# Zoz4/Pooraytracer

Hardware: AMD Instinct MI355X
Metric: Mrays/s (primary+secondary) at fixed spp; s/frame in ms_per_step (higher is better)
Workload: dtype f64; 1 GPU; cornell-box (synthetic stand-in, 20492 tris, 4-wide BVH 6148 nodes) 1024x1024 spp=500 depth=20 rr=0.8 bSampleLights seed=1; parallelism=32x32 tiles dealt diagonally over 1 GPU(s), rays_per_frame=2362685805

## Files before the change

pooraytracer_amd/csrc/prt_api.cpp:

```cpp
#include <hip/hip_runtime.h>
#include <rccl/rccl.h>

#include <algorithm>
#include <atomic>
#include <cmath>
#include <cstddef>
#include <cstdio>
#include <cstdlib>
#include <chrono>
#include <cstring>
#include <limits>
#include <map>
#include <memory>
#include <mutex>
#include <new>
#include <string>
#include <type_traits>
#include <vector>

#include "mesh_topology.h"
#include "prt_host.h"
#include "prt_launch.h"

namespace {
// ... 55 lines not shown
        if (e != hipSuccess || cap >= bytes) return e;
        if (done && (e = hipEventSynchronize(done.get())) != hipSuccess) return e;
        p.reset();
        cap = 0;
        if ((e = dev_alloc(p, bytes)) == hipSuccess) cap = bytes;
        return e;
    }
    hipError_t used(hipStream_t st) {
        const hipError_t e = done ? hipSuccess : make_event(done, hipEventDisableTiming);
        return e == hipSuccess ? hipEventRecord(done.get(), st) : e;
    }
    template <typename T>
    T* get() const { return static_cast<T*>(p.get()); }
};

struct Staging {
    std::vector<DevBuf<>> bufs;
    hipError_t e = hipSuccess;
    void* out(size_t bytes) {
        DevBuf<> b;
        if (e == hipSuccess) e = dev_alloc(b, std::max<size_t>(bytes, 16));
        bufs.push_back(std::move(b));
        return bufs.back().get();
    }
    void* in(const void* src, size_t bytes) {
        if (!src) return nullptr;
        void* d = out(bytes);
        if (e == hipSuccess) e = hipMemcpy(d, src, bytes, hipMemcpyHostToDevice);
        return d;
    }
    void sync(hipEvent_t ev = nullptr) {
        if (e == hipSuccess) e = ev ? hipEventSynchronize(ev) : hipDeviceSynchronize();
    }
    void down(void* dst, const void* src, size_t bytes) {
        if (e == hipSuccess) e = hipMemcpy(dst, src, bytes, hipMemcpyDeviceToHost);
    }
    int status(const std::string& who) const { return e == hipSuccess ? PRT_OK : hip_fail(who, e); }
};

template <typename R>
struct KernelConfig {
    DSceneT<R> d{};
    int blocks_per_cu[3] = {0, 0, 0};
    int blocks_per_cu_rays = 0;
    int light_lds = 0, ltri_lds = 0, mat_lds = 0;
    int stack_depth = PRT_STACK_DEPTH;
};
}

extern "C" int prt_dev_hooks(void) { return PRT_DEV_HOOKS; }

#if PRT_DEV_HOOKS
static std::atomic<int> g_render_form{PRT_RENDER_FORM_UNKNOWN};
static void note_render_form(bool plain) { g_render_form = plain ? PRT_RENDER_FORM_PLAIN : PRT_RENDER_FORM_GENERIC; }
extern "C" int prt_last_render_form(void) { return g_render_form; }
#else
static void note_render_form(bool) {}
extern "C" int prt_last_render_form(void) { return PRT_RENDER_FORM_UNKNOWN; }
#endif

#define PRT_HIP_AS(who, call)                                                                           \
    do {                                                                                                \
        const hipError_t e_ = (call);                                                                   \
        if (e_ != hipSuccess) return hip_fail(who, e_);                                                 \
    } while (0)
#define PRT_HIP(call) PRT_HIP_AS(#call, call)

struct PrtScene {
    std::vector<prt::HostTri> tris;
    std::vector<DMaterial> mats;
    std::vector<DTexture> texs;
    std::vector<double> texels_lin;
    size_t n_texel_reals = 0;
    size_t tex_footprint_bytes = 0;
    uint32_t tex_layouts = 0;
    prt::LightTree lights;
    prt::BuiltBVH bvh;
    std::vector<uint64_t> mesh_first;
    std::vector<int32_t> mesh_mat;
    std::vector<int32_t> light_meshes;
    bool explicit_lights = false;
    bool device_bvh = false;
    uint64_t generation = 0;
    PrtBvhInfo bvh_info{};
    int device = -1;
    int n_cu = 0;
    int blocks_wanted = 0;
    int feat = 0;
    KernelConfig<double> k64;
    KernelConfig<float> k32;
    bool f32_ready = false;
    int stack_need = PRT_STACK_DEPTH;
    const DNode* d_nodes_shallow = nullptr;
    uint32_t n_nodes_shallow = 0;
    std::vector<DevBuf<>> allocs;
    const uint32_t* d_order = nullptr;
    struct Refit {
        float* d_tbox = nullptr;
        uint32_t *d_parent = nullptr, *d_cnt = nullptr;
        uint32_t *d_parent_sh = nullptr, *d_cnt_sh = nullptr;
        void* d_scratch = nullptr;
        prt::RefitCheck* d_check = nullptr;
        double* d_sah = nullptr;
        Event ev0, ev1, ev2;
        Event done;
        bool pending = false;
        uint64_t count = 0;
    } refit;
    Scratch refit_in;
    bool host_stale = false;
    Event feat_done;
    bool feat_pending = false;
    bool dynamic_lights = false;
    struct LightArrays {
        void *nodes = nullptr, *tris = nullptr, *tab = nullptr, *nodes32 = nullptr, *tris32 = nullptr;
        size_t cap_nodes = 0, cap_tris = 0, cap_tab = 0, cap_nodes32 = 0, cap_tris32 = 0;
    };
    LightArrays light_res, light_spare;
    bool distance_queries = false;
    DTriCorners* d_corners = nullptr;
    bool signed_queries = false;
    prt::DSignedTables sq;
    size_t signed_bytes = 0;
    bool winding_queries = false;
    prt::DWindingMoment* d_moments = nullptr;
    struct LightUpdate {
        double* d_gather = nullptr;
        std::vector<double> h_gather;
        Scratch tmp;
        prt::LightTree next;
        prt::LightTablePlan plan;
        std::vector<uint32_t> words;
        uint32_t flag = 0;
        std::vector<DLightNodeT<float>> ln32;
        std::vector<DLightTriT<float>> lt32;
        std::vector<int32_t> prims;
        std::vector<prt::HostTri> saved;
        bool staged = false;
        bool staged_relaid = false, staged_dropped = false, staged_tables = false;
        Event g0, g1, t0, t1;
        bool tables_timed = false;
        uint64_t count = 0;
        double host_tree_ms = 0.0, gather_ms = 0.0;
        double staged_host_tree_ms = 0.0, staged_gather_ms = 0.0;
        int fail_alloc_at = -1, n_allocs = 0;
        uint32_t tables_dropped = 0, relaid = 0;
    } lu;
    hipError_t after_refit(hipStream_t st) const {
        return refit.pending ? hipStreamWaitEvent(st, refit.done.get(), 0) : hipSuccess;
    }
    struct CallSlot {
        DevBuf<DCounters> d_ctr;
        Scratch partial;
        Event ev0, ev1;
        Event done;
        bool timed = false;
        bool counted = false;
        uint64_t samples = 0;
        hipError_t start(hipStream_t st) {
            const hipError_t e = hipMemsetAsync(d_ctr.get(), 0, sizeof(DCounters), st);
            return e == hipSuccess ? hipEventRecord(ev0.get(), st) : e;
        }
        hipError_t stop(hipStream_t st) { return hipEventRecord(ev1.get(), st); }
        hipError_t finish(hipStream_t st, bool count, uint64_t n) {
            const hipError_t e = hipEventRecord(done.get(), st);
            if (e == hipSuccess) {
// ... 119 lines not shown
        sq = prt::DSignedTables();
        signed_bytes = 0;
        d_moments = nullptr;
        refit = Refit();
        light_res = light_spare = LightArrays();
        lu = LightUpdate();
        refit_in = Scratch();
        multi_fb = Scratch();
        sort = Scratch();
        dn = Scratch();
        for (CallSlot& q : slots) q = CallSlot();
        k64 = KernelConfig<double>();
        k32 = KernelConfig<float>();
        device = -1;
        f32_ready = false;
    }
};

static int check_node_count(const std::string& who, size_t n_nodes) {
    if (const char* e = dev_env("PRT_TEST_CLAIM_NODES")) n_nodes = (size_t)std::strtoull(e, nullptr, 10);
    std::string err;
    if (!prt::node_count_ok(n_nodes, &err)) return fail(PRT_E_LIMIT, who + ": " + err);
    return PRT_OK;
}

struct BvhDumpHeader {
    uint32_t magic, version;
    uint64_t n_tris, n_nodes;
    uint32_t built_on_device, depth;
    int32_t stack_need;
    uint32_t node_bytes;
    float grid_origin[3], grid_step[3], coord_scale;
    uint32_t zero;
};
static_assert(sizeof(BvhDumpHeader) == 72, "dump header layout");

static int dump_bvh(const char* path, const PrtScene* s, const DNode* nodes, size_t n_nodes, const uint32_t* order,
                    int stack_need) {
    BvhDumpHeader h;
    std::memset(&h, 0, sizeof(h));
    h.magic = 0x48564250u;
    h.version = 1;
    h.n_tris = s->tris.size();
    h.n_nodes = n_nodes;
    h.built_on_device = s->bvh_info.built_on_device;
    h.depth = s->bvh_info.depth;
    h.stack_need = stack_need;
    h.node_bytes = sizeof(DNode);
    for (int a = 0; a < 3; ++a) {
        h.grid_origin[a] = s->bvh.grid_origin[a];
        h.grid_step[a] = s->bvh.grid_step[a];
    }
    h.coord_scale = s->bvh.coord_scale;
    FILE* f = std::fopen(path, "wb");
    if (!f) return fail(PRT_E_INVALID, std::string("PRT_TEST_DUMP_BVH: cannot open ") + path);
    bool ok = std::fwrite(&h, sizeof(h), 1, f) == 1;
    ok = ok && std::fwrite(nodes, sizeof(DNode), n_nodes, f) == n_nodes;
    ok = ok && std::fwrite(order, sizeof(uint32_t), s->tris.size(), f) == s->tris.size();
    ok = (std::fclose(f) == 0) && ok;
    return ok ? PRT_OK : fail(PRT_E_INVALID, std::string("PRT_TEST_DUMP_BVH: cannot write ") + path);
}

template <typename T, typename U>
static void conv_arr(T* o, const U* a, int n) {
    for (int i = 0; i < n; ++i) o[i] = (T)a[i];
}

static void size_tables(const PrtScene* s, int budget, size_t mat_bytes, size_t ltri_bytes, size_t lnode_bytes, int* mat, int* ltri, int* light) {
    *mat = *ltri = *light = 0;
    const bool off = dev_env("PRT_TUNE_NO_LDS") && std::atoi(dev_env("PRT_TUNE_NO_LDS"));
    if (off || s->mats.empty() || s->mats.size() * mat_bytes > 8192 || (int)(s->mats.size() * mat_bytes) > budget) return;
    *mat = (int)s->mats.size();
    budget -= *mat * (int)mat_bytes;
    if (!s->lights.tris.empty() && s->lights.tris.size() <= 32 && (int)(s->lights.tris.size() * ltri_bytes) <= budget) {
        *ltri = (int)s->lights.tris.size();
        budget -= *ltri * (int)ltri_bytes;
    }
    *light = (int)std::min<size_t>(s->lights.nodes.size(), (size_t)(std::max(budget, 0) / (int)lnode_bytes));
    if (const char* e = dev_env("PRT_TUNE_LIGHT_LDS")) *light = std::min(*light, std::max(0, std::atoi(e)));
    if (const char* e = dev_env("PRT_TUNE_LTRI_LDS")) if (!std::atoi(e)) *ltri = 0;
}

template <typename R>
static bool frame_plain(const PrtScene* s, const KernelConfig<R>& k, bool count, bool rays, int jitter, int scramble, int sample_lights) {
    const auto plain = std::is_same<R, double>::value ? prt::render_plain : prt32::render_plain;
    return plain(s->feat, count, rays, k.d.n_lights, k.ltri_lds, jitter, scramble, sample_lights);
}
static bool generic_forced() {
    const char* e = dev_env("PRT_TUNE_GENERIC");
    return e && std::atoi(e);
}

template <typename R>
static int size_kernels(const PrtScene* s, KernelConfig<R>& k, bool drop_tables) {
    constexpr bool f64 = std::is_same<R, double>::value;
    const auto lds_budget = f64 ? prt::render_lds_budget : prt32::render_lds_budget;
    const auto table_bytes = f64 ? prt::render_table_bytes : prt32::render_table_bytes;
    const auto blocks_per_cu = f64 ? prt::render_blocks_per_cu : prt32::render_blocks_per_cu;
    size_tables(s, lds_budget(s->feat, k.stack_depth), sizeof(DMaterialT<R>), sizeof(DLightTriT<R>), sizeof(DLightNodeT<R>),
                &k.mat_lds, &k.ltri_lds, &k.light_lds);
    const bool pad = k.d.tri_stride == PRT_TRI_PAD_STRIDE(R) && sizeof(DTriT<R>) != PRT_TRI_PAD_STRIDE(R);
    const bool extra = !s->lights.tab.empty() || k.d.tex_compact != 0;
    auto blocks = [&](bool count, size_t tables, bool plain = false) { return blocks_per_cu(count, s->feat, tables, k.stack_depth, pad, extra, false, plain); };
    const size_t tables = table_bytes(k.light_lds, k.mat_lds, k.ltri_lds);
    k.blocks_per_cu[0] = blocks(false, tables);
    k.blocks_per_cu[2] = frame_plain(s, k, false, false, 0, 0, 1) ? blocks(false, tables, true) : 0;
    const int wanted = drop_tables && tables != 0 ? blocks(false, 0) : k.blocks_per_cu[0];
    if (k.blocks_per_cu[0] < wanted || (k.blocks_per_cu[2] && k.blocks_per_cu[2] < wanted)) {
        k.mat_lds = k.ltri_lds = k.light_lds = 0;
        k.blocks_per_cu[0] = wanted;
        k.blocks_per_cu[2] = 0;
    }
    k.blocks_per_cu[1] = blocks(true, table_bytes(k.light_lds, k.mat_lds, k.ltri_lds));
    if (dev_env("PRT_TUNE_VERBOSE")) {
        if (f64)
            std::fprintf(stderr, "[prt] fp64 render kernels: %d blocks per CU, LDS tables: %d materials, %d light triangles, %d light nodes\n",
                         k.blocks_per_cu[0], k.mat_lds, k.ltri_lds, k.light_lds);
        else
            std::fprintf(stderr, "[prt] fp32 render kernels: %d blocks per CU, stacks %d, LDS tables: %d materials, %d light triangles, %d light nodes\n",
                         k.blocks_per_cu[0], k.stack_depth, k.mat_lds, k.ltri_lds, k.light_lds);
    }
    return wanted;
}

static void size_kernels_again(PrtScene* s) {
    s->k64.blocks_per_cu_rays = 0;
    s->blocks_wanted = size_kernels(s, s->k64, true);
    if (s->f32_ready) {
        s->k32.blocks_per_cu_rays = 0;
        size_kernels(s, s->k32, false);
    }
}

template <typename R>
static int rays_blocks_per_cu(const PrtScene* s, KernelConfig<R>& k) {
    if (!k.blocks_per_cu_rays) {
        constexpr bool f64 = std::is_same<R, double>::value;
        const size_t tables = (f64 ? prt::render_table_bytes : prt32::render_table_bytes)(k.light_lds, k.mat_lds, k.ltri_lds);
        const bool pad = k.d.tri_stride == PRT_TRI_PAD_STRIDE(R) && sizeof(DTriT<R>) != PRT_TRI_PAD_STRIDE(R);
        k.blocks_per_cu_rays = (f64 ? prt::render_blocks_per_cu : prt32::render_blocks_per_cu)(false, s->feat, tables, k.stack_depth, pad, true, true, false);
    }
    return k.blocks_per_cu_rays;
}

template <typename R>
static uint32_t render_variant(const PrtScene* s, const KernelConfig<R>& k) {
    const bool llds = k.mat_lds != 0 || k.ltri_lds != 0 || k.light_lds != 0;
    const bool pad = k.d.tri_stride == PRT_TRI_PAD_STRIDE(R) && sizeof(DTriT<R>) != PRT_TRI_PAD_STRIDE(R);
    const bool extra = k.d.light_tab != nullptr || k.d.tex_compact != 0;
    return PRT_VARIANT_VALID | ((uint32_t)s->feat & PRT_VARIANT_PERM_MASK) | (llds ? PRT_VARIANT_LLDS : 0u) |
           (pad ? PRT_VARIANT_PAD : 0u) | (extra ? PRT_VARIANT_EXTRA : 0u);
}

struct TileLayout {
    int width, height, tile, tiles_x, tiles_y, n_tiles, rank, nranks, owned_tiles;
    uint64_t items_per_chunk;
    TileLayout(const PrtCamera& c, const PrtRenderParams& p) : width(c.width), height(c.height), rank(p.rank), nranks(p.nranks) {
        tile = p.tile_size > 0 ? p.tile_size : 32;
        tile = std::max(8, (tile + 7) / 8 * 8);
        tiles_x = (width + tile - 1) / tile;
        tiles_y = (height + tile - 1) / tile;
        n_tiles = tiles_x * tiles_y;
        owned_tiles = n_tiles > rank ? (n_tiles - rank + nranks - 1) / nranks : 0;
        items_per_chunk = (uint64_t)owned_tiles * tile * tile;
    }
    bool owns(int x, int y) const {
        const int tx = x / tile, ty = y / tile;
        const int kx = ((tx - 3 * ty) % tiles_x + tiles_x) % tiles_x;
        return (ty * tiles_x + kx) % nranks == rank;
    }
    uint64_t owned_pixels() const {
        uint64_t px = 0;
        for (int k = rank; k < n_tiles; k += nranks) {
            const int ty = k / tiles_x, tx = (k - ty * tiles_x + 3 * ty) % tiles_x;
            px += (uint64_t)std::max(0, std::min(tile, width - tx * tile)) * (uint64_t)std::max(0, std::min(tile, height - ty * tile));
        }
        return px;
    }
    void set(DRenderParams& P) const {
        P.tile = tile; P.tiles_x = tiles_x; P.tiles_y = tiles_y; P.n_tiles = n_tiles;
        P.rank = rank; P.nranks = nranks; P.owned_tiles = owned_tiles; P.items_per_chunk = items_per_chunk;
    }
};

#ifndef PRT_CHAIN_MIN_DEFAULT
#define PRT_CHAIN_MIN_DEFAULT 8
#endif
static DRenderParams base_params(const PrtScene* s, const PrtRenderParams* p) {
    DRenderParams P;
// ... 15 lines not shown
    P.stack_depth = PRT_STACK_DEPTH;
    return P;
}

static DRenderParamsT<float> to_f32(const DRenderParams& P, const KernelConfig<float>& k) {
    static_assert(sizeof(DRenderParamsT<float>) == 400, "DRenderParamsT changed: convert its new fields here");
    DRenderParamsT<float> o;
    std::memset(&o, 0, sizeof(o));
    o.spp = P.spp; o.max_depth = P.max_depth; o.sample_lights = P.sample_lights; o.chunks = P.chunks;
    o.rr = (float)P.rr; o.inv_rr = (float)P.inv_rr;
    conv_arr(o.background, P.background, 3);
    o.seed_key = P.seed_key;
    o.tile = P.tile; o.tiles_x = P.tiles_x; o.tiles_y = P.tiles_y; o.n_tiles = P.n_tiles;
    o.rank = P.rank; o.nranks = P.nranks; o.owned_tiles = P.owned_tiles; o.jitter = P.jitter;
    o.keep = P.keep; o.leaf_batch = P.leaf_batch; o.inner_min = P.inner_min; o.scramble = P.scramble; o.cached_min = P.cached_min; o.chain_min = P.chain_min;
    o.light_lds = k.light_lds; o.mat_lds = k.mat_lds; o.ltri_lds = k.ltri_lds;
    o.stack_depth = k.stack_depth;
    o.items_per_chunk = P.items_per_chunk; o.n_items = P.n_items;
    std::memcpy(o.chunk_begin, P.chunk_begin, sizeof(P.chunk_begin));
    return o;
}
static DCameraT<float> to_f32(const DCamera& C) {
    DCameraT<float> o;
    conv_arr(o.center, C.center, 3); conv_arr(o.pixel00, C.pixel00, 3);
    conv_arr(o.du, C.du, 3); conv_arr(o.dv, C.dv, 3);
    o.width = C.width; o.height = C.height;
    return o;
}

extern "C" {

int prt_abi_version(void) { return PRT_ABI_VERSION; }
const char* prt_last_error(void) { return g_err.c_str(); }

int prt_device_count(int* n) {
    if (!n) return fail(PRT_E_INVALID, "prt_device_count: null argument");
    int c = 0;
    hipError_t e = hipGetDeviceCount(&c);
    if (e != hipSuccess) {
        *n = 0;
        return fail(PRT_E_NO_DEVICE, std::string("hipGetDeviceCount: ") + hipGetErrorString(e));
    }
    *n = c;
    return PRT_OK;
}

int prt_scene_create(const PrtSceneDesc* desc, PrtScene** out) {
    if (!desc || !out) return fail(PRT_E_INVALID, "prt_scene_create: null argument");
    *out = nullptr;
    if (desc->n_tris && !desc->vertices) return fail(PRT_E_INVALID, "prt_scene_create: vertices is null");
    if (desc->n_meshes && (!desc->mesh_first_tri || !desc->mesh_material))
        return fail(PRT_E_INVALID, "prt_scene_create: mesh arrays are null");
    if (desc->n_materials && !desc->materials) return fail(PRT_E_INVALID, "prt_scene_create: materials is null");
    if (desc->n_textures && !desc->textures) return fail(PRT_E_INVALID, "prt_scene_create: textures is null");
    if (desc->n_meshes) {
        if (desc->mesh_first_tri[0] != 0 || desc->mesh_first_tri[desc->n_meshes] != desc->n_tris)
            return fail(PRT_E_INVALID, "prt_scene_create: mesh_first_tri must start at 0 and end at n_tris");
        for (uint32_t m = 0; m < desc->n_meshes; ++m) {
            if (desc->mesh_first_tri[m] > desc->mesh_first_tri[m + 1])
                return fail(PRT_E_INVALID, "prt_scene_create: mesh_first_tri must be ascending");
            if (desc->mesh_material[m] < 0 || (uint32_t)desc->mesh_material[m] >= desc->n_materials)
                return fail(PRT_E_INVALID, "prt_scene_create: mesh_material out of range");
        }
    } else if (desc->n_tris) {
        return fail(PRT_E_INVALID, "prt_scene_create: triangles without meshes");
    }
    if (desc->n_light_meshes && !desc->light_meshes) return fail(PRT_E_INVALID, "prt_scene_create: light_meshes is null");
    for (uint32_t i = 0; i < (desc->light_meshes ? desc->n_light_meshes : 0u); ++i)
        if (desc->light_meshes[i] < 0 || (uint32_t)desc->light_meshes[i] >= desc->n_meshes)
            return fail(PRT_E_INVALID, "prt_scene_create: light_meshes entry out of range");
    for (uint32_t i = 0; i < desc->n_materials; ++i) {
        const PrtMaterial& m = desc->materials[i];
        if (m.type < PRT_MAT_LAMBERTIAN || m.type > PRT_MAT_EMPTY)
            return fail(PRT_E_INVALID, "prt_scene_create: unknown material type");
        if (m.texture >= (int32_t)desc->n_textures) return fail(PRT_E_INVALID, "prt_scene_create: texture index out of range");
    }
    for (uint64_t i = 0; i < desc->n_tris * 9; ++i)
        if (!(std::fabs(desc->vertices[i]) <= 1e18))
            return fail(PRT_E_INVALID, "prt_scene_create: vertex coordinate is not finite (or beyond 1e18)");
    PrtScene* s = new (std::nothrow) PrtScene();
    if (!s) return fail(PRT_E_OOM, "prt_scene_create: out of host memory");
    try {
        prt::setup_triangles(*desc, s->tris);
        s->mesh_first.assign(desc->mesh_first_tri, desc->mesh_first_tri + (desc->n_meshes ? desc->n_meshes + 1 : 0));
        s->mesh_mat.assign(desc->mesh_material, desc->mesh_material + desc->n_meshes);
        s->explicit_lights = desc->light_meshes != nullptr;
        if (s->explicit_lights) s->light_meshes.assign(desc->light_meshes, desc->light_meshes + desc->n_light_meshes);
        prt::setup_materials(*desc, s->mats);
        s->texs.resize(desc->n_textures);
        for (uint32_t i = 0; i < desc->n_textures; ++i) {
            const PrtTexture& t = desc->textures[i];
            DTexture& o = s->texs[i];
            o.width = t.width;
            o.height = t.height;
            o.channels = t.channels;
            o.has_data = (t.data && t.width > 0 && t.height > 0 && t.channels > 0) ? 1 : 0;
            o.offset = s->texels_lin.size();
            if (o.has_data) {
                double lut[256];
                for (int b = 0; b < 256; ++b) {
                    const double c = (1.0 / 255.0) * b;
                    lut[b] = (c <= 0.04045) ? c * (1. / 12.92) : std::pow((c + 0.055) * (1. / 1.055), 2.4);
                }
                const size_t npx = (size_t)t.width * t.height;
                s->texels_lin.reserve(s->texels_lin.size() + npx * 3);
                for (size_t i = 0; i < npx; ++i) {
                    const uint8_t* px = t.data + i * t.channels;
                    if (t.channels >= 3) {
                        s->texels_lin.push_back(lut[px[0]]);
                        s->texels_lin.push_back(lut[px[1]]);
                        s->texels_lin.push_back(lut[px[2]]);
                    } else {
                        const double g = (1.0 / 255.0) * px[0];
                        s->texels_lin.insert(s->texels_lin.end(), {g, g, g});
                    }
                }
            }
        }
        prt::build_light_tree(*desc, s->tris, s->mats, s->lights);
        s->device_bvh = (desc->flags & PRT_SCENE_DEVICE_BVH) && s->tris.size() >= 2;
        if (!s->device_bvh) {
            std::string err;
            const auto t0 = std::chrono::steady_clock::now();
            if (!prt::build_bvh(s->tris, s->bvh, &err)) {
                delete s;
                return fail(PRT_E_LIMIT, "prt_scene_create: " + err);
            }
            if (const int rc = check_node_count("prt_scene_create", s->bvh.nodes.size())) {
                delete s;
                return rc;
            }
            s->bvh_info.build_ms = std::chrono::duration<double, std::milli>(std::chrono::steady_clock::now() - t0).count();
        }
    } catch (const std::bad_alloc&) {
        delete s;
        return fail(PRT_E_OOM, "prt_scene_create: out of host memory");
    } catch (const std::exception& e) {
        delete s;
        return fail(PRT_E_INVALID, std::string("prt_scene_create: ") + e.what());
    }
    s->last.bvh_nodes = s->bvh.nodes.size();
    s->last.bvh_depth = s->bvh.depth;
    s->bvh_info.n_nodes = s->bvh.nodes.size();
    s->bvh_info.depth = s->bvh.depth;
    if (const char* p = dev_env("PRT_TEST_DUMP_BVH"))
        if (!s->device_bvh) {
            const int rc = dump_bvh(p, s, s->bvh.nodes.data(), s->bvh.nodes.size(), s->bvh.order.data(), s->bvh.stack_need);
            if (rc != PRT_OK) {
                delete s;
                return rc;
            }
        }
    *out = s;
    return PRT_OK;
}

void prt_scene_destroy(PrtScene* s) {
    if (!s) return;
    s->release();
    delete s;
}

int prt_scene_bvh_info(const PrtScene* s, PrtBvhInfo* out) {
    if (!s || !out) return fail(PRT_E_INVALID, "prt_scene_bvh_info: null argument");
    *out = s->bvh_info;
    out->node_bytes = (uint32_t)sizeof(DNode);
// ... 300 lines not shown
            for (int y0 = 0; y0 < t.height; ++y0)
                for (int x0 = 0; x0 < t.width; ++x0) {
                    const int x1 = std::min(x0 + 1, t.width - 1), y1 = std::min(y0 + 1, t.height - 1);
                    double* o = quads.data() + at;
                    const int tap[4][2] = {{x0, y0}, {x1, y0}, {x0, y1}, {x1, y1}};
                    for (int k = 0; k < 4; ++k) std::memcpy(o + 3 * k, px + ((size_t)tap[k][1] * t.width + tap[k][0]) * 3, 24);
                    at += 16;
                }
        }
        d.tex_compact = compact ? 1u : 0u;
        s->tex_footprint_bytes = compact ? 0 : cells_all * 16 * sizeof(double);
        s->tex_layouts = cells_all == 0 ? 0u : (compact ? 2u : 1u);
        s->n_texel_reals = quads.size();
        if ((rc = s->up(qt, &d.textures))) return rc;
        if ((rc = s->up(quads, &d.texels_lin))) return rc;
    }
    if ((rc = s->up(s->lights.nodes, &d.light_nodes))) return rc;
    d.light_tab = nullptr;
    if (!s->lights.tab.empty() && (rc = s->up(s->lights.tab, &d.light_tab))) return rc;
    if ((rc = s->up(s->lights.tris, &d.light_tris))) return rc;
    s->light_res.nodes = const_cast<DLightNode*>(d.light_nodes);
    s->light_res.tris = const_cast<DLightTri*>(d.light_tris);
    s->light_res.tab = const_cast<uint32_t*>(d.light_tab);
    s->light_res.cap_nodes = s->lights.nodes.size();
    s->light_res.cap_tris = s->lights.tris.size();
    s->light_res.cap_tab = s->lights.tab.size();
    d.light_root = s->lights.root;
    d.n_lights = (int32_t)s->lights.tris.size();
    d.light_area = s->lights.area;
    d.n_tris = (uint32_t)n;
    for (PrtScene::CallSlot& q : s->slots) {
        PRT_HIP_AS("hipMalloc", dev_alloc(q.d_ctr, sizeof(DCounters)));
        PRT_HIP(hipMemset(q.d_ctr.get(), 0, sizeof(DCounters)));
        PRT_HIP(make_event(q.ev0, hipEventDefault));
        PRT_HIP(make_event(q.ev1, hipEventDefault));
        PRT_HIP(make_event(q.done, hipEventDisableTiming));
    }
    s->feat = 0;
    for (const DMaterial& m : s->mats) {
        if (m.texture >= 0) s->feat |= 1;
        if (m.type == PRT_MAT_PHONG) s->feat |= 2;
        if (m.type == PRT_MAT_COOKTORRANCE) s->feat |= 4;
    }
    if (const char* e = dev_env("PRT_TUNE_FEAT")) s->feat |= std::atoi(e);
    s->feat = prt::render_permutation(s->feat);
    {
        int need = s->bvh.stack_need;
        if (s->bvh_info.built_on_device)
            PRT_HIP_AS("hipMemcpy(hn.data(), d.nodes, (size_t)d.n_nodes * sizeof(DNode), hipMemcpyDeviceToHost)",
                       device_tree_stack_need(d.nodes, d.n_nodes, &need));
        if (dump_path && (rc = dump_bvh(dump_path, s, dump_nodes.data(), dump_nodes.size(), dump_order.data(), need))) return rc;
        s->set_stack_need(need);
        s->d_nodes_shallow = nullptr;
        s->n_nodes_shallow = 0;
        if (dev_env("PRT_TUNE_VERBOSE")) std::fprintf(stderr, "[prt] tree needs %d stack entries\n", s->stack_need);
    }
    static_assert(sizeof(DLightNode) == 16 && sizeof(DLightTri) % 16 == 0, "LDS staging copies 16-byte pieces");
    s->blocks_wanted = size_kernels(s, s->k64, true);
    if (s->distance_queries && (rc = corners_from_host(s, "prt_scene_upload"))) return rc;
    if (s->signed_queries && (rc = signed_from_host(s, "prt_scene_upload"))) return rc;
    if (s->winding_queries && (rc = winding_from_resident(s, "prt_scene_upload"))) return rc;
    return PRT_OK;
}

static void light_desc(const PrtScene* s, PrtSceneDesc& d) {
    std::memset(&d, 0, sizeof(d));
    d.n_tris = s->tris.size();
    d.n_meshes = (uint32_t)s->mesh_mat.size();
    d.mesh_first_tri = s->mesh_first.data();
    d.mesh_material = s->mesh_mat.data();
    static const int32_t none = 0;
    d.light_meshes = s->explicit_lights ? (s->light_meshes.empty() ? &none : s->light_meshes.data()) : nullptr;
    d.n_light_meshes = (uint32_t)s->light_meshes.size();
}

int prt_scene_update_vertices(PrtScene* s, const double* vertices, const double* normals) {
    if (!s || (!vertices && !s->tris.empty())) return fail(PRT_E_INVALID, "prt_scene_update_vertices: null argument");
    for (size_t i = 0; i < s->tris.size() * 9; ++i)
        if (!(std::fabs(vertices[i]) <= 1e18)) return fail(PRT_E_INVALID, "prt_scene_update_vertices: vertex coordinate is not finite (or beyond 1e18)");
    ++s->generation;
    try {
        prt::update_triangles(vertices, normals, s->tris);
        s->host_stale = false;
        PrtSceneDesc d;
        light_desc(s, d);
        s->lights = prt::LightTree();
        prt::build_light_tree(d, s->tris, s->mats, s->lights);
        if (s->device >= 0 && s->tris.size() >= 2) {
            s->device_bvh = true;
        } else if (!s->device_bvh) {
            std::string err;
            const auto t0 = std::chrono::steady_clock::now();
            if (!prt::build_bvh(s->tris, s->bvh, &err)) return fail(PRT_E_LIMIT, "prt_scene_update_vertices: " + err);
            s->bvh_info.build_ms = std::chrono::duration<double, std::milli>(std::chrono::steady_clock::now() - t0).count();
            s->last.bvh_nodes = s->bvh_info.n_nodes = s->bvh.nodes.size();
            s->last.bvh_depth = s->bvh_info.depth = s->bvh.depth;
            if (const char* p = dev_env("PRT_TEST_DUMP_BVH")) {
                const int rc = dump_bvh(p, s, s->bvh.nodes.data(), s->bvh.nodes.size(), s->bvh.order.data(), s->bvh.stack_need);
                if (rc != PRT_OK) return rc;
            }
        }
    } catch (const std::bad_alloc&) {
        return fail(PRT_E_OOM, "prt_scene_update_vertices: out of host memory");
    }
    if (s->device >= 0) return prt_scene_upload(s, s->device);
    return PRT_OK;
}

static int ensure_f32_impl(PrtScene* s);
static int f32_stack_depth(int need) {
    int depth = need <= PRT_STACK_SHALLOW ? PRT_STACK_SHALLOW : PRT_STACK_DEPTH;
    if (const char* e = dev_env("PRT_TUNE_STACK32")) depth = std::max(need, std::min(PRT_STACK_DEPTH, std::atoi(e)));
    return depth;
}
static void light_tables_f32(const prt::LightTree& lights, std::vector<DLightNodeT<float>>& ln, std::vector<DLightTriT<float>>& lt) {
    ln.resize(lights.nodes.size());
    for (size_t i = 0; i < ln.size(); ++i) {
        std::memset(&ln[i], 0, sizeof(ln[i]));
        ln[i].left_area = (float)lights.nodes[i].left_area;
        ln[i].left = lights.nodes[i].left;
        ln[i].right = lights.nodes[i].right;
    }
    lt.resize(lights.tris.size());
    for (size_t i = 0; i < lt.size(); ++i) {
        const DLightTri& a = lights.tris[i];
        DLightTriT<float>& o = lt[i];
        std::memset(&o, 0, sizeof(o));
        conv_arr(o.v0, a.v0, 3); conv_arr(o.v1, a.v1, 3); conv_arr(o.v2, a.v2, 3); conv_arr(o.n, a.n, 3);
        o.area = (float)a.area; o.material = a.material; o.prim = a.prim; o.pdf = (float)a.pdf;
    }
}
static int ensure_f32(PrtScene* s) {
    if (s->f32_ready) return PRT_OK;
    const size_t mark = s->allocs.size();
    const int rc = ensure_f32_impl(s);
    if (rc != PRT_OK) {
        KeepError keep;
        s->allocs.resize(mark);
        s->k32 = KernelConfig<float>();
        s->light_res.nodes32 = s->light_res.tris32 = nullptr;
        s->light_res.cap_nodes32 = s->light_res.cap_tris32 = 0;
    }
    return rc;
}
static int ensure_f32_impl(PrtScene* s) {
    const DScene& d = s->k64.d;
    KernelConfig<float>& k = s->k32;
    DSceneT<float>& f = k.d;
    const size_t n = d.n_tris;
    const uint32_t stride = d.tri_stride == sizeof(DTriT<double>) ? (uint32_t)sizeof(DTriT<float>) : PRT_TRI_PAD_STRIDE(float);
    void *t = nullptr, *sh = nullptr, *tx = nullptr;
    int rc;
    if ((rc = s->alloc(n * (size_t)stride, &t)) || (rc = s->alloc(n * sizeof(DTriShadeT<float>), &sh)) ||
        (rc = s->alloc(s->n_texel_reals * sizeof(float), &tx)))
        return rc;
    PRT_HIP(s->after_refit(nullptr));
    prt32::launch_convert_tris(d.tris, d.tri_stride, (uint32_t)n, t, stride, nullptr);
    prt32::launch_convert_shade(d.shade, (uint32_t)n, static_cast<DTriShadeT<float>*>(sh), nullptr);
    prt32::launch_convert_reals(d.texels_lin, s->n_texel_reals, static_cast<float*>(tx), nullptr);
    PRT_HIP(hipGetLastError());
    std::vector<DMaterialT<float>> mats(s->mats.size());
    for (size_t i = 0; i < mats.size(); ++i) {
        const DMaterial& a = s->mats[i];
        DMaterialT<float>& o = mats[i];
        std::memset(&o, 0, sizeof(o));
        o.type = a.type; o.texture = a.texture;
// ... 21 lines not shown
    {
        int need = s->stack_need;
        if ((rc = s->shallow_resident())) return rc;
        if (s->d_nodes_shallow) need = std::min(need, PRT_STACK_SHALLOW);
        s->share_with_f32();
        k.stack_depth = f32_stack_depth(need);
        if (dev_env("PRT_TUNE_VERBOSE")) std::fprintf(stderr, "[prt] fp32 tables: tree needs %d stack entries, using %d\n", need, k.stack_depth);
    }
    size_kernels(s, k, false);
    s->f32_ready = true;
    return PRT_OK;
}

static int require_uploaded(PrtScene* s, const char* who) {
    if (!s) return fail(PRT_E_INVALID, std::string(who) + ": null scene");
    if (s->device < 0) return fail(PRT_E_NO_DEVICE, std::string(who) + ": scene is not uploaded to a HIP device (no CPU path exists)");
    PRT_HIP(hipSetDevice(s->device));
    return PRT_OK;
}

namespace {
float f32_round_down(double v) {
    float f = (float)v;
    if ((double)f > v) f = std::nextafter(f, -std::numeric_limits<float>::infinity());
    return f;
}
float f32_round_up(double v) {
    float f = (float)v;
    if ((double)f < v) f = std::nextafter(f, std::numeric_limits<float>::infinity());
    return f;
}
size_t round16(size_t b) { return (b + 15) & ~(size_t)15; }
}

static hipError_t refit_baseline(PrtScene* s, hipStream_t st) {
    const PrtScene::Refit& R = s->refit;
    const DScene& d = s->k64.d;
    prt::launch_refit_parents(d.nodes, d.n_nodes, R.d_parent, st);
    prt::launch_refit_sah(d.nodes, d.n_nodes, d.grid_origin, d.grid_step, R.d_scratch, R.d_sah, st);
    return hipMemcpyAsync(R.d_sah + 1, R.d_sah, sizeof(double), hipMemcpyDeviceToDevice, st);
}

static int refit_prepare(PrtScene* s, hipStream_t st) {
    PrtScene::Refit& R = s->refit;
    const DScene& d = s->k64.d;
    int rc;
    if (!R.d_check) {
        void *tbox, *parent, *cnt, *scratch, *check, *sah;
        if ((rc = s->alloc((size_t)d.n_tris * 6 * sizeof(float), &tbox)) || (rc = s->alloc((size_t)d.n_nodes * sizeof(uint32_t), &parent)) ||
            (rc = s->alloc(round16((size_t)d.n_nodes * sizeof(uint32_t)), &cnt)) || (rc = s->alloc(prt::refit_scratch_bytes(), &scratch)) ||
            (rc = s->alloc(2 * sizeof(double), &sah)) || (rc = s->alloc(sizeof(prt::RefitCheck), &check)))
            return rc;
        PRT_HIP(make_event(R.ev0, hipEventDefault));
        PRT_HIP(make_event(R.ev1, hipEventDefault));
        PRT_HIP(make_event(R.ev2, hipEventDefault));
        PRT_HIP(make_event(R.done, hipEventDisableTiming));
        if ((rc = s->shallow_resident())) return rc;
        R.d_tbox = static_cast<float*>(tbox);
        R.d_parent = static_cast<uint32_t*>(parent);
        R.d_cnt = static_cast<uint32_t*>(cnt);
        R.d_scratch = scratch;
        R.d_sah = static_cast<double*>(sah);
        PRT_HIP_AS("hipMemcpyAsync(R.d_sah + 1, R.d_sah, sizeof(double), hipMemcpyDeviceToDevice, st)", refit_baseline(s, st));
        PRT_HIP(hipGetLastError());
        R.d_check = static_cast<prt::RefitCheck*>(check);
    }
    if (s->d_nodes_shallow && !R.d_parent_sh) {
        void *parent, *cnt;
        if ((rc = s->alloc((size_t)s->n_nodes_shallow * sizeof(uint32_t), &parent)) ||
            (rc = s->alloc(round16((size_t)s->n_nodes_shallow * sizeof(uint32_t)), &cnt)))
            return rc;
        prt::launch_refit_parents(s->d_nodes_shallow, s->n_nodes_shallow, static_cast<uint32_t*>(parent), st);
        PRT_HIP(hipGetLastError());
        R.d_cnt_sh = static_cast<uint32_t*>(cnt);
        R.d_parent_sh = static_cast<uint32_t*>(parent);
    }
    return PRT_OK;
}

struct RefitGridHost {
    float origin[3], step[3], root_hi[3];
    double origin_d[3], delta;
    bool lights_moved = false;
};

static int refit_begin(PrtScene* s, const std::string& who, const double* d_verts, const double* d_normals, hipStream_t st,
                       RefitGridHost& g) {
    DScene& d = s->k64.d;
    const uint32_t n = d.n_tris;
    PrtScene::Refit& R = s->refit;
    if (!d_verts) return fail(PRT_E_INVALID, who + ": null vertices");
    PRT_HIP_AS(who, s->after_refit(st));
    {
        const size_t mark = s->allocs.size();
        const bool fresh = !R.d_check;
        const DNode* const shallow_before = s->d_nodes_shallow;
        const uint32_t n_shallow_before = s->n_nodes_shallow;
        const int rc = refit_prepare(s, st);
        if (rc != PRT_OK) {
            KeepError keep;
            if (fresh) {
                (void)hipDeviceSynchronize();
                s->allocs.resize(mark);
                R = PrtScene::Refit();
                s->d_nodes_shallow = shallow_before;
                s->n_nodes_shallow = n_shallow_before;
            }
            return rc;
        }
    }
    PrtScene::LightUpdate& U = s->lu;
    const size_t nl = (size_t)d.n_lights;
    const bool gather = s->dynamic_lights && nl > 0;
    if (gather && !U.d_gather) {
        PRT_HIP_AS(who, make_event(U.g0, hipEventDefault));
        PRT_HIP_AS(who, make_event(U.g1, hipEventDefault));
        PRT_HIP_AS(who, make_event(U.t0, hipEventDefault));
        PRT_HIP_AS(who, make_event(U.t1, hipEventDefault));
        void* p = nullptr;
        if (const int rc = s->alloc(nl * 18 * sizeof(double), &p)) return rc;
        U.d_gather = static_cast<double*>(p);
    }
    if (gather) {
        try {
            U.h_gather.resize(nl * 18);
        } catch (const std::bad_alloc&) {
            return fail(PRT_E_OOM, who + ": out of host memory");
        }
        PRT_HIP_AS(who, hipEventRecord(U.g0.get(), st));
    }
    prt::launch_refit_check(d_verts, n, d.light_tris, (uint32_t)d.n_lights, R.d_scratch, R.d_check, st, d_normals,
                            gather ? U.d_gather : nullptr, gather ? U.d_gather + nl * 9 : nullptr);
    PRT_HIP_AS(who, hipGetLastError());
    prt::RefitCheck c;
    PRT_HIP_AS(who, hipMemcpyAsync(&c, R.d_check, sizeof(c), hipMemcpyDeviceToHost, st));
    if (gather) {
        PRT_HIP_AS(who, hipMemcpyAsync(U.h_gather.data(), U.d_gather, nl * (d_normals ? 18 : 9) * sizeof(double), hipMemcpyDeviceToHost, st));
        PRT_HIP_AS(who, hipEventRecord(U.g1.get(), st));
    }
    PRT_HIP_AS(who, hipEventRecord(R.done.get(), st));
    R.pending = true;
    PRT_HIP_AS(who, hipStreamSynchronize(st));
    if (c.flags & 1u) return fail(PRT_E_INVALID, who + ": vertex coordinate is not finite (or beyond 1e18)");
    if ((c.flags & 2u) && !s->dynamic_lights)
        return fail(PRT_E_INVALID, who + ": a vertex of a light mesh moved; emitters stay in place under a refit (the light tree is not "
                                         "rebuilt) - use prt_scene_update_vertices");
    g.lights_moved = (c.flags & 2u) != 0;
    const double extent = std::max(1.0, std::max(c.hi[0] - c.lo[0], std::max(c.hi[1] - c.lo[1], c.hi[2] - c.lo[2])));
    g.delta = 1e-9 * extent + 256.0 * std::numeric_limits<double>::epsilon() * c.scale;
    for (int a = 0; a < 3; ++a) {
        g.origin[a] = f32_round_down(c.lo[a] - 2.0 * g.delta);
        g.origin_d[a] = (double)g.origin[a];
        g.root_hi[a] = f32_round_up((c.hi[a] + g.delta) - g.origin_d[a]);
    }
    const float zero[3] = {0.f, 0.f, 0.f};
    float rel0[3];
    prt::quant_grid(zero, g.root_hi, false, rel0, g.step);
    return PRT_OK;
}

static int light_grow(PrtScene* s, void*& p, size_t& cap, size_t need, size_t elem) {
    if (p && cap >= need) return PRT_OK;
    if (s->lu.n_allocs++ == s->lu.fail_alloc_at) return fail(PRT_E_OOM, "light update: injected allocation failure (PRT_TEST_FAIL_LIGHT_STAGE)");
    (void)s->take(p);
    p = nullptr;
    cap = 0;
    if (const int rc = s->alloc(need * elem, &p)) return rc;
    cap = need;
    return PRT_OK;
}

static void light_unstage(PrtScene* s) {
    PrtScene::LightUpdate& U = s->lu;
    if (!U.staged) return;
    for (size_t l = U.prims.size(); l-- > 0;) s->tris[(size_t)U.prims[l]] = U.saved[l];
    U.staged = false;
}

static int light_stage(PrtScene* s, const std::string& who, bool normals, hipStream_t st) {
    PrtScene::LightUpdate& U = s->lu;
    const size_t nl = s->lights.tris.size();
    const auto t0 = std::chrono::steady_clock::now();
    bool tables = false;
    try {
        U.prims.resize(nl);
        U.saved.resize(nl);
        for (size_t l = 0; l < nl; ++l) {
            U.prims[l] = s->lights.tris[l].prim;
            U.saved[l] = s->tris[(size_t)U.prims[l]];
        }
        U.staged = true;
        prt::update_triangles_listed(U.prims.data(), nl, U.h_gather.data(), normals ? U.h_gather.data() + nl * 9 : nullptr, s->tris);
        PrtSceneDesc ld;
        light_desc(s, ld);
        U.next = prt::LightTree();
        prt::build_light_tree(ld, s->tris, s->mats, U.next, false);
        tables = prt::plan_light_tables(U.next, U.plan);
        if (tables) U.words.assign(U.plan.tab.size(), 0u);
    } catch (const std::bad_alloc&) {
        light_unstage(s);
        return fail(PRT_E_OOM, who + ": out of host memory");
    }
    U.staged_host_tree_ms = std::chrono::duration<double, std::milli>(std::chrono::steady_clock::now() - t0).count();
    U.n_allocs = 0;
    U.fail_alloc_at = dev_env("PRT_TEST_FAIL_LIGHT_STAGE") ? std::atoi(dev_env("PRT_TEST_FAIL_LIGHT_STAGE")) : -1;
    {
        float ms = 0.f;
        U.staged_gather_ms = hipEventElapsedTime(&ms, U.g0.get(), U.g1.get()) == hipSuccess ? ms : 0.0;
    }
    auto failed = [&](int rc) {
        KeepError keep;
        light_unstage(s);
        return rc;
    };
    if (U.next.tris.size() != nl) return failed(fail(PRT_E_INVALID, who + ": the set of light triangles changed"));
    PrtScene::LightArrays& A = s->light_spare;
    const size_t n_full = U.next.full_nodes.size(), n_words = tables ? U.plan.tab.size() : 0, n_tab = tables ? U.plan.node.size() : 0;
    int rc;
    if ((rc = light_grow(s, A.nodes, A.cap_nodes, n_full, sizeof(DLightNode))) || (rc = light_grow(s, A.tris, A.cap_tris, nl, sizeof(DLightTri))) ||
        (n_words && (rc = light_grow(s, A.tab, A.cap_tab, n_words, sizeof(uint32_t)))))
        return failed(rc);
    if (s->f32_ready && ((rc = light_grow(s, A.nodes32, A.cap_nodes32, n_full, sizeof(DLightNodeT<float>))) ||
                         (rc = light_grow(s, A.tris32, A.cap_tris32, nl, sizeof(DLightTriT<float>)))))
        return failed(rc);
    const size_t off_full = 16, off_area = off_full + n_full * sizeof(DLightNode), off_node = off_area + n_tab * sizeof(double);
    auto hip = [&](hipError_t e) { return e == hipSuccess ? PRT_OK : failed(hip_fail(who, e)); };
    if ((rc = hip(U.tmp.reserve(off_node + n_tab * sizeof(int32_t), st)))) return rc;
    char* const tmp = U.tmp.get<char>();
    auto put = [&](void* dst, const void* src, size_t bytes) { return bytes ? hipMemcpyAsync(dst, src, bytes, hipMemcpyHostToDevice, st) : hipSuccess; };
    const std::vector<DLightNode>& top = tables ? U.plan.top : U.next.full_nodes;
// ... 23 lines not shown
        B.total = (float)U.next.area;
        if ((rc = hip(hipEventRecord(U.t0.get(), st))) || (rc = hip(prt::launch_light_tables(B, st))) ||
            (rc = hip(hipMemcpyAsync(&U.flag, B.flag, sizeof(uint32_t), hipMemcpyDeviceToHost, st))) ||
            (rc = hip(hipMemcpyAsync(U.words.data(), A.tab, n_words * sizeof(uint32_t), hipMemcpyDeviceToHost, st))) ||
            (rc = hip(hipEventRecord(U.t1.get(), st))) || (rc = hip(U.tmp.used(st))) || (rc = hip(hipStreamSynchronize(st))))
            return rc;
        U.tables_timed = true;
        dropped = U.flag != 0 || (dev_env("PRT_TEST_FAIL_LIGHT_VERIFY") && std::atoi(dev_env("PRT_TEST_FAIL_LIGHT_VERIFY")));
        if (dropped) {
            if ((rc = hip(put(A.nodes, U.next.full_nodes.data(), n_full * sizeof(DLightNode))))) return rc;
        } else {
            try {
                prt::apply_light_tables(U.next, U.plan, U.words);
            } catch (const std::bad_alloc&) {
                return failed(fail(PRT_E_OOM, who + ": out of host memory"));
            }
        }
    }
    if (s->f32_ready) {
        try {
            light_tables_f32(U.next, U.ln32, U.lt32);
        } catch (const std::bad_alloc&) {
            return failed(fail(PRT_E_OOM, who + ": out of host memory"));
        }
        if ((rc = hip(put(A.nodes32, U.ln32.data(), U.ln32.size() * sizeof(DLightNodeT<float>)))) ||
            (rc = hip(put(A.tris32, U.lt32.data(), U.lt32.size() * sizeof(DLightTriT<float>)))))
            return rc;
    }
    const prt::LightTree& old = s->lights;
    bool relaid = old.nodes.size() != U.next.nodes.size() || old.tab.size() != U.next.tab.size() || old.root != U.next.root ||
                  old.n_tables != U.next.n_tables;
    for (size_t t = 0; !relaid && t < U.next.n_tables; ++t)
        relaid = std::memcmp(old.tab.data() + 8 * t, U.next.tab.data() + 8 * t, 5 * sizeof(uint32_t)) != 0;
    U.staged_relaid = relaid;
    U.staged_dropped = dropped;
    U.staged_tables = tables;
    return PRT_OK;
}

static void light_commit(PrtScene* s) {
    PrtScene::LightUpdate& U = s->lu;
    if (!U.staged) return;
    U.staged = false;
    std::swap(s->light_res, s->light_spare);
    const PrtScene::LightArrays& A = s->light_res;
    s->lights = std::move(U.next);
    U.next = prt::LightTree();
    DScene& d = s->k64.d;
    d.light_nodes = static_cast<const DLightNode*>(A.nodes);
    d.light_tris = static_cast<const DLightTri*>(A.tris);
    d.light_tab = s->lights.tab.empty() ? nullptr : static_cast<const uint32_t*>(A.tab);
    d.light_root = s->lights.root;
    d.n_lights = (int32_t)s->lights.tris.size();
    d.light_area = s->lights.area;
    if (s->f32_ready) {
        DSceneT<float>& f = s->k32.d;
        f.light_nodes = static_cast<const DLightNodeT<float>*>(A.nodes32);
        f.light_tris = static_cast<const DLightTriT<float>*>(A.tris32);
        s->share_with_f32();
    }
    ++U.count;
    U.host_tree_ms = U.staged_host_tree_ms;
    U.gather_ms = U.staged_gather_ms;
    U.relaid = U.staged_relaid ? 1u : 0u;
    U.tables_dropped = U.staged_dropped ? 1u : 0u;
    if (U.staged_relaid) size_kernels_again(s);
}

static int lights_then_readers(PrtScene* s, const std::string& who, bool lights_moved, bool normals, hipStream_t st) {
    if (lights_moved)
        if (const int rc = light_stage(s, who, normals, st)) return rc;
    hipError_t e = hipSuccess;
    for (PrtScene::CallSlot& q : s->slots)
        if (q.timed && e == hipSuccess) e = hipStreamWaitEvent(st, q.done.get(), 0);
    if (s->feat_pending && e == hipSuccess) e = hipStreamWaitEvent(st, s->feat_done.get(), 0);
    if (e != hipSuccess) {
        light_unstage(s);
        return hip_fail(who, e);
    }
    light_commit(s);
    return PRT_OK;
}

static void refit_commit_grid(PrtScene* s, const float origin[3], const float step[3], float coord_scale) {
    s->set_grid(origin, step, coord_scale);
    ++s->generation;
}

static int dump_resident_bvh(PrtScene* s, const std::string& who, hipStream_t st) {
    const char* path = dev_env("PRT_TEST_DUMP_BVH");
    if (!path) return PRT_OK;
    const DScene& d = s->k64.d;
    std::vector<DNode> hn(d.n_nodes);
    std::vector<uint32_t> ho(d.n_tris);
    PRT_HIP_AS(who, hipStreamSynchronize(st));
    PRT_HIP_AS(who, hipMemcpy(hn.data(), d.nodes, hn.size() * sizeof(DNode), hipMemcpyDeviceToHost));
    PRT_HIP_AS(who, hipMemcpy(ho.data(), s->d_order, ho.size() * sizeof(uint32_t), hipMemcpyDeviceToHost));
    return dump_bvh(path, s, hn.data(), hn.size(), ho.data(), s->stack_need);
}

static void launch_position_followers(PrtScene* s, const double* d_verts, const double* d_normals, const RefitGridHost& g, hipStream_t st) {
    const DScene& d = s->k64.d;
    const uint32_t n = d.n_tris;
    prt::launch_refit_tris(d_verts, d_normals, s->d_order, n, const_cast<DTri*>(d.tris), d.tri_stride, const_cast<DTriShade*>(d.shade),
                           s->refit.d_tbox, g.origin_d, g.delta, st);
    if (s->d_corners) prt::launch_gather_corners(d_verts, s->d_order, n, s->d_corners, st);
    if (s->d_corners && s->sq.slot) prt::launch_pseudonormals(s->d_corners, s->sq, st);
    if (s->f32_ready) {
        const DSceneT<float>& f = s->k32.d;
        prt32::launch_convert_tris(d.tris, d.tri_stride, n, const_cast<DTriT<float>*>(f.tris), f.tri_stride, st);
        prt32::launch_convert_shade(d.shade, n, const_cast<DTriShadeT<float>*>(f.shade), st);
    }
}

static hipError_t launch_tree_followers(PrtScene* s, hipStream_t st) {
    const DScene& d = s->k64.d;
    if (!s->d_moments || !s->d_corners) return hipSuccess;
    return prt::launch_winding_moments(d.nodes, d.n_nodes, s->refit.d_parent, s->refit.d_cnt, s->d_corners, d.n_tris, s->d_moments, st);
}

static int refit_impl(PrtScene* s, const std::string& who, const double* d_verts, const double* d_normals, hipStream_t st) {
    DScene& d = s->k64.d;
    const uint32_t n = d.n_tris;
    if (n == 0) return PRT_OK;
    PrtScene::Refit& R = s->refit;
    RefitGridHost g;
    if (const int rc = refit_begin(s, who, d_verts, d_normals, st, g)) return rc;
    const float *origin = g.origin, *step = g.step;
    if (const int rc = lights_then_readers(s, who, g.lights_moved, d_normals != nullptr, st)) return rc;
    {
        float cs = std::max(g.root_hi[0], std::max(g.root_hi[1], g.root_hi[2]));
        if (s->bvh_info.built_on_device)
            for (int a = 0; a < 3; ++a) cs = std::max(cs, (float)(65535.0 * (double)step[a]));
        refit_commit_grid(s, origin, step, std::nextafter(cs, std::numeric_limits<float>::infinity()));
    }
    PRT_HIP_AS(who, hipEventRecord(R.ev0.get(), st));
    launch_position_followers(s, d_verts, d_normals, g, st);
    PRT_HIP_AS(who, hipGetLastError());
    PRT_HIP_AS(who, hipEventRecord(R.ev1.get(), st));
    PRT_HIP_AS(who, prt::launch_refit_boxes(const_cast<DNode*>(d.nodes), d.n_nodes, R.d_parent, R.d_cnt, R.d_tbox, n, step, st));
    if (s->d_nodes_shallow)
        PRT_HIP_AS(who, prt::launch_refit_boxes(const_cast<DNode*>(s->d_nodes_shallow), s->n_nodes_shallow, R.d_parent_sh, R.d_cnt_sh,
                                                R.d_tbox, n, step, st));
    PRT_HIP_AS(who, launch_tree_followers(s, st));
    prt::launch_refit_sah(d.nodes, d.n_nodes, origin, step, R.d_scratch, R.d_sah + 1, st);
    PRT_HIP_AS(who, hipGetLastError());
    PRT_HIP_AS(who, hipEventRecord(R.ev2.get(), st));
    PRT_HIP_AS(who, hipEventRecord(R.done.get(), st));
    ++R.count;
    return dump_resident_bvh(s, who, st);
}

static int rebuild_impl(PrtScene* s, const std::string& who, const double* d_verts, const double* d_normals, hipStream_t st) {
    DScene& d = s->k64.d;
    const uint32_t n = d.n_tris;
    if (n < 2) return refit_impl(s, who, d_verts, d_normals, st);
    PrtScene::Refit& R = s->refit;
    RefitGridHost g;
    if (const int rc = refit_begin(s, who, d_verts, d_normals, st, g)) return rc;
    const int fail_at = dev_env("PRT_TEST_FAIL_REBUILD") ? std::atoi(dev_env("PRT_TEST_FAIL_REBUILD")) : -1;
    int n_allocs = 0;
    auto injected = [&]() { return n_allocs++ == fail_at; };
    auto alloc = [&](size_t bytes, DevBuf<>& out) -> int {
        if (injected()) return fail(PRT_E_OOM, who + ": injected allocation failure (PRT_TEST_FAIL_REBUILD)");
        PRT_HIP_AS(who, dev_alloc(out, std::max<size_t>(bytes, 256)));
        return PRT_OK;
    };
    DevBuf<> boxes, nodes, order, shade, inv, parent, cnt, moments;
    int rc;
    if ((rc = alloc((size_t)n * sizeof(prt::PrimBox), boxes))) return rc;
    prt::launch_prim_boxes(d_verts, n, static_cast<float*>(boxes.get()), g.origin_d, g.delta, st);
    PRT_HIP_AS(who, hipGetLastError());
    prt::DeviceBVH db;
    {
        if (injected()) return fail(PRT_E_OOM, who + ": injected allocation failure (PRT_TEST_FAIL_REBUILD)");
        std::string err;
        if (!prt::build_bvh_device_boxes(static_cast<const prt::PrimBox*>(boxes.get()), g.origin, n, db, &err, st))
            return fail(PRT_E_HIP, who + ": " + err);
        nodes.reset(db.d_nodes);
        order.reset(db.d_order);
    }
    if ((rc = check_node_count(who, db.n_nodes))) return rc;
    if ((rc = alloc((size_t)n * sizeof(DTriShade), shade)) || (rc = alloc((size_t)n * sizeof(uint32_t), inv)) ||
        (rc = alloc((size_t)db.n_nodes * sizeof(uint32_t), parent)) || (rc = alloc(round16((size_t)db.n_nodes * sizeof(uint32_t)), cnt)))
        return rc;
    if (s->d_moments && (rc = alloc((size_t)db.n_nodes * 4 * sizeof(prt::DWindingMoment), moments))) return rc;
    int need = PRT_STACK_DEPTH;
    try {
        PRT_HIP_AS(who, device_tree_stack_need(db.d_nodes, db.n_nodes, &need));
    } catch (const std::bad_alloc&) {
        return fail(PRT_E_OOM, who + ": out of host memory");
    }
    if ((rc = lights_then_readers(s, who, g.lights_moved, d_normals != nullptr, st))) return rc;

    refit_commit_grid(s, db.grid_origin, db.grid_step, db.coord_scale);
    const DTriShade* const shade_old = d.shade;
    const uint32_t* const order_old = s->d_order;
    DevBuf<> old[9] = {s->take(d.nodes),  s->take(s->d_order),        s->take(d.shade),      s->take(R.d_parent),
                       s->take(R.d_cnt),  s->take(s->d_nodes_shallow), s->take(R.d_parent_sh), s->take(R.d_cnt_sh),
                       s->take(moments ? s->d_moments : nullptr)};
    s->adopt_device_tree(db);
    d.shade = static_cast<const DTriShade*>(shade.get());
    R.d_parent = static_cast<uint32_t*>(parent.get());
    R.d_cnt = static_cast<uint32_t*>(cnt.get());
    R.d_parent_sh = R.d_cnt_sh = nullptr;
    s->d_nodes_shallow = nullptr;
    s->n_nodes_shallow = 0;
    if (moments) s->d_moments = static_cast<prt::DWindingMoment*>(moments.get());
    for (DevBuf<>* b : {&nodes, &order, &shade, &parent, &cnt, &moments})
        if (*b) s->allocs.push_back(std::move(*b));
    s->device_bvh = true;
    s->set_stack_need(need);
    if (s->f32_ready) {
        s->share_with_f32();
        s->k32.stack_depth = f32_stack_depth(s->stack_need);
    }
    size_kernels_again(s);
    prt::launch_permute_shade(shade_old, order_old, s->d_order, n, static_cast<uint32_t*>(inv.get()), const_cast<DTriShade*>(d.shade), st);
    launch_position_followers(s, d_verts, d_normals, g, st);
    PRT_HIP_AS(who, refit_baseline(s, st));
    PRT_HIP_AS(who, launch_tree_followers(s, st));
    PRT_HIP_AS(who, hipGetLastError());
    PRT_HIP_AS(who, hipEventRecord(R.done.get(), st));
    PRT_HIP_AS(who, hipStreamSynchronize(st));
    return dump_resident_bvh(s, who, st);
}

static int host_positions(PrtScene* s, const char* name, const double* vertices, const double* normals, bool rebuild) {
    const std::string who = name;
    int rc = require_uploaded(s, name);
    if (rc) return rc;
    const size_t n = s->tris.size(), bytes = n * 9 * sizeof(double);
    if (n == 0) return PRT_OK;
    if (!vertices) return fail(PRT_E_INVALID, who + ": null vertices");
    PRT_HIP_AS(who, s->refit_in.reserve(bytes * (normals ? 2 : 1), nullptr));
    double* dv = s->refit_in.get<double>();
    double* dn = normals ? dv + n * 9 : nullptr;
    PRT_HIP(hipMemcpyAsync(dv, vertices, bytes, hipMemcpyHostToDevice, nullptr));
    if (normals) PRT_HIP(hipMemcpyAsync(dn, normals, bytes, hipMemcpyHostToDevice, nullptr));
    rc = (rebuild ? rebuild_impl : refit_impl)(s, who, dv, dn, nullptr);
    PRT_HIP_AS(who, s->refit_in.used(nullptr));
    if (rc != PRT_OK) {
        KeepError keep;
        (void)hipStreamSynchronize(nullptr);
        return rc;
    }
    try {
        prt::update_triangles(vertices, normals, s->tris);
        s->host_stale = false;
        if (!s->device_bvh) {
            if (n >= 2) s->device_bvh = true;
            else {
                std::string err;
                if (!prt::build_bvh(s->tris, s->bvh, &err)) return fail(PRT_E_LIMIT, who + ": " + err);
            }
        }
    } catch (const std::bad_alloc&) {
        s->host_stale = true;
        return fail(PRT_E_OOM, who + ": out of host memory (the resident scene holds the new geometry)");
    }
    return PRT_OK;
}

int prt_scene_refit(PrtScene* s, const double* vertices, const double* normals) {
    return host_positions(s, "prt_scene_refit", vertices, normals, false);
}

int prt_scene_rebuild(PrtScene* s, const double* vertices, const double* normals) {
    return host_positions(s, "prt_scene_rebuild", vertices, normals, true);
}

static int device_positions(PrtScene* s, const char* name, const void* d_vertices, const void* d_normals, void* stream, bool rebuild) {
    int rc = require_uploaded(s, name);
    if (rc) return rc;
    rc = (rebuild ? rebuild_impl : refit_impl)(s, name, static_cast<const double*>(d_vertices), static_cast<const double*>(d_normals),
                                               reinterpret_cast<hipStream_t>(stream));
    if (rc == PRT_OK && !s->tris.empty()) s->host_stale = true;
    return rc;
// ... 650 lines not shown
    pass.spp = p->spp;
    pass.first = sample_begin;
    pass.rays = true;
    pass.d_rays = d_rays;
    pass.d_keys = d_keys;
    pass.n_rays = n;
    return render_impl(s, who, nullptr, p, pass, d_rgb_f64, d_rgb_f32, 0, reinterpret_cast<hipStream_t>(stream));
}

int prt_ray_color(PrtScene* s, const PrtRay* rays, const uint32_t* keys, size_t n, const PrtRenderParams* p, int32_t sample_begin,
                  double* rgb_f64, float* rgb_f32) {
    const char* who = "prt_ray_color";
    int rc = require_uploaded(s, who);
    if (rc) return rc;
    if (n && !rays) return fail(PRT_E_INVALID, "prt_ray_color: null ray buffer");
    if (n >= 0xffffffffULL) return fail(PRT_E_LIMIT, "prt_ray_color: more than 2^32 work items (rays x sample chunks) in one launch");
    for (size_t i = 0; i < n; ++i) {
        const PrtRay& r = rays[i];
        bool ok = r.d[0] != 0.0 || r.d[1] != 0.0 || r.d[2] != 0.0;
        for (int a = 0; a < 3; ++a) ok = ok && std::isfinite(r.o[a]) && std::isfinite(r.d[a]);
        if (!ok) return fail(PRT_E_INVALID, "prt_ray_color: ray " + std::to_string(i) + " has a non-finite origin or direction, or a zero direction");
    }
    Staging b;
    void* dr = b.in(rays, n * sizeof(PrtRay));
    void* dk = b.in(keys, n * sizeof(uint32_t));
    void* d64 = rgb_f64 ? b.out(n * 3 * sizeof(double)) : nullptr;
    void* d32 = rgb_f32 ? b.out(n * 3 * sizeof(float)) : nullptr;
    if ((rc = b.status(who)) || (rc = prt_ray_color_device(s, dr, dk, n, p, sample_begin, d64, d32, nullptr)))
        return rc;
    b.sync();
    if (rgb_f64) b.down(rgb_f64, d64, n * 3 * sizeof(double));
    if (rgb_f32) b.down(rgb_f32, d32, n * 3 * sizeof(float));
    return b.status(who);
}

int prt_render_device(PrtScene* s, const PrtCamera* cam, const PrtRenderParams* p, void* d_rgb_f64, void* d_rgb_f32,
                      int count_work, void* stream) {
    int rc = require_uploaded(s, "prt_render_device");
    if (rc) return rc;
    if (!cam || !p) return fail(PRT_E_INVALID, "prt_render_device: null argument");
    if (cam->width < 1 || cam->height < 1) return fail(PRT_E_INVALID, "prt_render_device: bad image size");
    if (p->spp < 1) return fail(PRT_E_INVALID, "prt_render_device: spp must be >= 1");
    RenderPass pass;
    pass.spp = p->spp;
    return render_impl(s, "prt_render_device", cam, p, pass, d_rgb_f64, d_rgb_f32, count_work, reinterpret_cast<hipStream_t>(stream));
}

static int render_impl(PrtScene* s, const char* who, const PrtCamera* cam, const PrtRenderParams* p, const RenderPass& pass,
                       void* d_rgb_f64, void* d_rgb_f32, int count_work, hipStream_t st) {
    int rc = PRT_OK;
    const std::string w(who);
    if (p->precision != PRT_PRECISION_F64 && p->precision != PRT_PRECISION_F32) return fail(PRT_E_INVALID, w + ": unsupported precision");
    const bool f32 = p->precision == PRT_PRECISION_F32;
    if (f32 && (rc = ensure_f32(s))) return rc;
    if (!pass.rays && (p->nranks < 1 || p->rank < 0 || p->rank >= p->nranks)) return fail(PRT_E_INVALID, w + ": bad rank/nranks");

    DCamera C;
    if (pass.rays) std::memset(&C, 0, sizeof(C));
    else prt::setup_camera(*cam, C);
    DRenderParams P = base_params(s, p);
    P.spp = pass.d_sum ? 1 : pass.spp;
    P.cached_min = 24;
    if (const char* e = dev_env("PRT_TUNE_CACHED_MIN")) P.cached_min = std::max(1, std::atoi(e));
    if (const char* e = dev_env("PRT_TUNE_CHAIN_MIN")) P.chain_min = std::min(65, std::max(1, std::atoi(e)));
    if (const char* e = dev_env("PRT_TUNE_KEEP")) P.keep = std::min(64, std::max(0, std::atoi(e)));
    if (const char* e = dev_env("PRT_TUNE_LEAF_BATCH")) P.leaf_batch = std::min(64, std::max(1, std::atoi(e)));
    if (const char* e = dev_env("PRT_TUNE_INNER_MIN")) P.inner_min = std::min(64, std::max(0, std::atoi(e)));
    if (const char* e = dev_env("PRT_TUNE_SCRAMBLE")) P.scramble = std::atoi(e) ? 1 : 0;
    uint64_t owned_pixels = pass.n_rays;
    if (pass.rays) {
        P.scramble = 0;
        P.tile = 8; P.tiles_x = P.tiles_y = P.n_tiles = 1; P.rank = 0; P.nranks = 1; P.owned_tiles = 1;
        P.items_per_chunk = pass.n_rays;
    } else {
        const TileLayout L(*cam, *p);
        L.set(P);
        owned_pixels = L.owned_pixels();
    }
    if (pass.d_list) {
        P.scramble = PRT_ITEMS_FROM_LIST;
        P.items_per_chunk = pass.list_n;
    }
    const bool count = count_work != 0;
    const bool plain = !generic_forced() && (f32 ? frame_plain(s, s->k32, count, pass.rays, P.jitter, P.scramble, P.sample_lights)
                                                 : frame_plain(s, s->k64, count, pass.rays, P.jitter, P.scramble, P.sample_lights));
    int bpc = (f32 ? s->k32.blocks_per_cu : s->k64.blocks_per_cu)[count ? 1 : plain ? 2 : 0];
    if (pass.rays) bpc = f32 ? rays_blocks_per_cu(s, s->k32) : rays_blocks_per_cu(s, s->k64);
    const uint64_t lanes = (uint64_t)s->n_cu * bpc * PRT_BLOCK;
    std::vector<int> sizes;
    const int spp = pass.spp;
    int want = p->sample_chunks;
    if (const char* e = dev_env("PRT_TUNE_CHUNKS")) want = std::atoi(e);
    if (pass.d_list) {
        for (int c = 0; c < spp / pass.batch; ++c) sizes.push_back(pass.batch);
    } else if (want > 0) {
        want = std::min(want, std::min(spp, PRT_MAX_CHUNKS));
        for (int c = 0; c < want; ++c) sizes.push_back((int)(((int64_t)(c + 1) * spp) / want - ((int64_t)c * spp) / want));
    } else if (P.items_per_chunk == 0) {
        sizes.push_back(spp);
    } else {
        int body = P.items_per_chunk < 2 * lanes ? 64 : 128;
        if (const char* e = dev_env("PRT_TUNE_BODY")) body = std::max(1, std::atoi(e));
        body = std::max(body, (spp + PRT_MAX_CHUNKS / 2 - 1) / (PRT_MAX_CHUNKS / 2));
        double var = 4.0;
        if (const char* e = dev_env("PRT_TUNE_VAR")) var = std::max(0.25, std::atof(e));
        double c = ((double)P.items_per_chunk / (double)lanes) / var;
        for (;;) {
            sizes.clear();
            int64_t sum = 0;
            while (sum < spp && (int)sizes.size() <= PRT_MAX_CHUNKS) {
                int64_t sz = (int64_t)std::floor(c * (double)sum);
                sz = std::max<int64_t>(1, std::min<int64_t>(sz, body));
                sz = std::min<int64_t>(sz, spp - sum);
                sizes.push_back((int)sz);
                sum += sz;
            }
            if ((int)sizes.size() <= PRT_MAX_CHUNKS) break;
            c *= 1.25;
            if (c > 1e9) body *= 2;
        }
        std::reverse(sizes.begin(), sizes.end());
    }
    sizes.erase(std::remove(sizes.begin(), sizes.end(), 0), sizes.end());
    if (sizes.empty()) sizes.push_back(spp);
    int chunks = (int)sizes.size();
    P.chunk_begin[0] = pass.first;
    for (int c = 0; c < chunks; ++c) P.chunk_begin[c + 1] = P.chunk_begin[c] + sizes[c];
    P.chunks = chunks;
    P.n_items = P.items_per_chunk * (uint64_t)chunks;
    if (P.n_items >= 0xffffffffULL) return fail(PRT_E_LIMIT, w + ": more than 2^32 work items (pixels x sample chunks) in one launch");

    const size_t need = std::max<size_t>(P.n_items * 3, 3);
    hipError_t we;
    PrtScene::CallSlot& q = *s->next_slot(st, &we);
    PRT_HIP(we);
    PRT_HIP(q.partial.reserve(need * sizeof(double), st));
    double* d_partial = q.partial.get<double>();
    const size_t npx = pass.rays ? (size_t)pass.n_rays * 3 : (size_t)C.width * C.height * 3;
    DevBuf<> dump_buf;
    unsigned long long dump_cap = 0;
    std::string dump_path;
    if (d_rgb_f64 && npx) PRT_HIP(hipMemsetAsync(d_rgb_f64, 0, npx * sizeof(double), st));
    if (d_rgb_f32 && npx) PRT_HIP(hipMemsetAsync(d_rgb_f32, 0, npx * sizeof(float), st));
    PRT_HIP(q.start(st));
    if (P.max_depth < 0) P.n_items = 0;
    if (P.n_items) {
        const uint64_t want = (P.n_items + PRT_BLOCK - 1) / PRT_BLOCK;
        const unsigned grid = (unsigned)std::max<uint64_t>(1, std::min<uint64_t>(want, (uint64_t)s->n_cu * bpc));
        PRT_HIP(q.set_pointers(st, pass.d_list, nullptr));
        if (pass.rays) PRT_HIP(q.set_rays(st, pass.d_rays, pass.d_keys));
        if (const char* e = dev_env("PRT_TUNE_DUMP_RAYS")) {
            const std::string v(e);
            const size_t comma = v.find(',');
            if (count && comma != std::string::npos) {
                dump_cap = std::strtoull(v.substr(0, comma).c_str(), nullptr, 10);
                dump_path = v.substr(comma + 1);
                PRT_HIP(dev_alloc(dump_buf, (size_t)dump_cap * sizeof(PrtRay)));
                const unsigned long long vals[3] = {(unsigned long long)(uintptr_t)dump_buf.get(), dump_cap, 0ULL};
                PRT_HIP(hipMemcpyAsync(reinterpret_cast<char*>(q.d_ctr.get()) + offsetof(DCounters, ray_dump), vals, sizeof(vals), hipMemcpyHostToDevice, st));
            }
        }
        if (f32) prt32::launch_render(s->k32.d, to_f32(C), to_f32(P, s->k32), d_partial, q.d_ctr.get(), count, s->feat, grid, st, pass.rays, plain);
        else prt::launch_render(s->k64.d, C, P, d_partial, q.d_ctr.get(), count, s->feat, grid, st, pass.rays, plain);
        note_render_form(plain);
        PRT_HIP(hipGetLastError());
    }
    PRT_HIP(q.stop(st));
    if (dump_buf) {
        PRT_HIP(hipStreamSynchronize(st));
        DCounters h;
        PRT_HIP(hipMemcpy(&h, q.d_ctr.get(), sizeof(h), hipMemcpyDeviceToHost));
        const size_t nd = (size_t)std::min<unsigned long long>(h.ray_dump_n, dump_cap);
        std::vector<PrtRay> rays(nd);
        PRT_HIP(hipMemcpy(rays.data(), dump_buf.get(), nd * sizeof(PrtRay), hipMemcpyDeviceToHost));
        dump_buf.reset();
        if (FILE* f = std::fopen(dump_path.c_str(), "wb")) {
            std::fwrite(rays.data(), sizeof(PrtRay), nd, f);
            std::fclose(f);
        }
        std::fprintf(stderr, "[prt] dumped %zu of %llu rays to %s\n", nd, h.ray_dump_n, dump_path.c_str());
    }
    if (pass.d_list) {
        if (!P.n_items) PRT_HIP(hipMemsetAsync(d_partial, 0, need * sizeof(double), st));
        prt::launch_accumulate_list(P, d_partial, pass.d_list, (uint32_t)pass.batch, (uint32_t)spp, pass.d_sum, pass.d_moment,
                                    pass.d_count, st);
        PRT_HIP(hipGetLastError());
    } else if (P.n_items) {
        if (pass.rays) prt::launch_finalize_rays(P, d_partial, static_cast<double*>(d_rgb_f64), static_cast<float*>(d_rgb_f32), st);
        else if (pass.d_sum) prt::launch_accumulate(C, P, d_partial, pass.d_sum, st);
        else prt::launch_finalize(C, P, d_partial, static_cast<double*>(d_rgb_f64), static_cast<float*>(d_rgb_f32), st);
        PRT_HIP(hipGetLastError());
    }
    const uint64_t samples = !P.n_items ? 0 : pass.d_list ? (uint64_t)pass.list_n * (uint64_t)spp : owned_pixels * (uint64_t)spp;
    PRT_HIP(q.finish(st, count, samples));
    return PRT_OK;
}

int prt_render(PrtScene* s, const PrtCamera* cam, const PrtRenderParams* p, double* rgb_f64, float* rgb_f32) {
    int rc = require_uploaded(s, "prt_render");
    if (rc) return rc;
    if (!cam || !p) return fail(PRT_E_INVALID, "prt_render: null argument");
    if (cam->width < 1 || cam->height < 1) return fail(PRT_E_INVALID, "prt_render: bad image size");
    const size_t npx = (size_t)cam->width * cam->height * 3;
    Staging b;
    void* d64 = rgb_f64 ? b.out(npx * sizeof(double)) : nullptr;
    void* d32 = rgb_f32 ? b.out(npx * sizeof(float)) : nullptr;
    if ((rc = b.status("prt_render")) || (rc = prt_render_device(s, cam, p, d64, d32, 0, nullptr))) return rc;
    b.sync();
    if (rgb_f64) b.down(rgb_f64, d64, npx * sizeof(double));
    if (rgb_f32) b.down(rgb_f32, d32, npx * sizeof(float));
    return b.status("prt_render");
}

int prt_render_samples(PrtScene* s, const PrtCamera* cam, const PrtRenderParams* p, const int32_t* pixel_xy, size_t n_pixels,
                       int32_t sample_begin, int32_t sample_count, double* radiance, int32_t* trace) {
    const char* who = "prt_render_samples";
    int rc = require_uploaded(s, who);
    if (rc) return rc;
    if (!cam || !p || (n_pixels && (!pixel_xy || !radiance))) return fail(PRT_E_INVALID, "prt_render_samples: null argument");
    if (cam->width < 1 || cam->height < 1) return fail(PRT_E_INVALID, "prt_render_samples: bad image size");
    if (p->precision != PRT_PRECISION_F64) return fail(PRT_E_INVALID, "prt_render_samples: fp64 only");
    if (sample_begin < 0 || sample_count < 0) return fail(PRT_E_INVALID, "prt_render_samples: bad sample range");
    if (n_pixels == 0 || sample_count == 0) return PRT_OK;
    if (n_pixels * (size_t)PRT_MAX_CHUNKS >= 0xffffffffULL) return fail(PRT_E_LIMIT, "prt_render_samples: too many pixels");
    std::vector<int32_t> pix(n_pixels);
    for (size_t k = 0; k < n_pixels; ++k) {
        const int32_t i = pixel_xy[2 * k], j = pixel_xy[2 * k + 1];
        if (i < 0 || j < 0 || i >= cam->width || j >= cam->height) return fail(PRT_E_INVALID, "prt_render_samples: pixel outside the image");
        pix[k] = j * cam->width + i;
    }
    DCamera C;
    prt::setup_camera(*cam, C);
    DRenderParams P = base_params(s, p);
    P.spp = 1;
    P.scramble = PRT_ITEMS_FROM_LIST;
    P.cached_min = 65;
    P.tile = 8; P.tiles_x = P.tiles_y = P.n_tiles = 1; P.rank = 0; P.nranks = 1; P.owned_tiles = 1;
    P.items_per_chunk = n_pixels;
    const bool count = trace != nullptr;
    const bool plain = !generic_forced() && frame_plain(s, s->k64, count, false, P.jitter, P.scramble, P.sample_lights);
    const int bpc = s->k64.blocks_per_cu[count ? 1 : plain ? 2 : 0];
    const size_t per_launch = n_pixels * (size_t)std::min<int>(sample_count, PRT_MAX_CHUNKS);
    Staging b;
    const int32_t* d_pix = static_cast<const int32_t*>(b.in(pix.data(), n_pixels * sizeof(int32_t)));
    double* d_part = static_cast<double*>(b.out(per_launch * 3 * sizeof(double)));
    int32_t* d_trace = trace ? static_cast<int32_t*>(b.out(per_launch * PRT_TRACE_WORDS * sizeof(int32_t))) : nullptr;
    if ((rc = b.status(who))) return rc;
    std::vector<double> part(per_launch * 3);
    std::vector<int32_t> tr(trace ? per_launch * PRT_TRACE_WORDS : 0);
    for (int32_t s0 = 0; s0 < sample_count; s0 += PRT_MAX_CHUNKS) {
        const int chunks = std::min<int>(PRT_MAX_CHUNKS, sample_count - s0);
        for (int c = 0; c <= chunks; ++c) P.chunk_begin[c] = sample_begin + s0 + c;
        P.chunks = chunks;
        P.n_items = P.items_per_chunk * (uint64_t)chunks;
        hipError_t we;
        PrtScene::CallSlot& q = *s->next_slot(nullptr, &we);
        PRT_HIP_AS(who, we);
        const uint64_t want = (P.n_items + PRT_BLOCK - 1) / PRT_BLOCK;
        const unsigned grid = (unsigned)std::max<uint64_t>(1, std::min<uint64_t>(want, (uint64_t)s->n_cu * bpc));
        if (d_trace) PRT_HIP_AS(who, hipMemset(d_trace, 0, (size_t)P.n_items * PRT_TRACE_WORDS * sizeof(int32_t)));
        PRT_HIP_AS(who, q.start(nullptr));
        PRT_HIP_AS(who, q.set_pointers(nullptr, d_pix, d_trace));
        if (P.max_depth >= 0) {
            prt::launch_render(s->k64.d, C, P, d_part, q.d_ctr.get(), count, s->feat, grid, nullptr, false, plain);
            note_render_form(plain);
        } else PRT_HIP_AS(who, hipMemset(d_part, 0, (size_t)P.n_items * 3 * sizeof(double)));
        PRT_HIP_AS(who, hipGetLastError());
        PRT_HIP_AS(who, q.stop(nullptr));
        PRT_HIP_AS(who, q.finish(nullptr, count, P.max_depth >= 0 ? P.n_items : 0));
        PRT_HIP_AS(who, hipDeviceSynchronize());
        PRT_HIP_AS(who, hipMemcpy(part.data(), d_part, (size_t)P.n_items * 3 * sizeof(double), hipMemcpyDeviceToHost));
        if (trace) PRT_HIP_AS(who, hipMemcpy(tr.data(), d_trace, (size_t)P.n_items * PRT_TRACE_WORDS * sizeof(int32_t), hipMemcpyDeviceToHost));
        for (int c = 0; c < chunks; ++c)
            for (size_t k = 0; k < n_pixels; ++k) {
                const size_t item = (size_t)c * n_pixels + k, o = k * (size_t)sample_count + (size_t)(s0 + c);
                std::memcpy(radiance + o * 3, part.data() + item * 3, 3 * sizeof(double));
                if (trace) std::memcpy(trace + o * PRT_TRACE_WORDS, tr.data() + item * PRT_TRACE_WORDS, PRT_TRACE_WORDS * sizeof(int32_t));
            }
    }
    return PRT_OK;
}

namespace {
struct CommSet {
    std::vector<ncclComm_t> comms;
};
std::mutex g_comm_mutex;
std::map<std::vector<int>, CommSet> g_comms;
}

namespace {
struct DeviceGuard {
    int dev = -1;
    DeviceGuard() { if (hipGetDevice(&dev) != hipSuccess) dev = -1; }
    ~DeviceGuard() { if (dev >= 0) (void)hipSetDevice(dev); }
};
void drop_comms_locked(std::map<std::vector<int>, CommSet>::iterator it, bool abort) {
    for (ncclComm_t c : it->second.comms)
        if (c) (void)(abort ? ncclCommAbort(c) : ncclCommDestroy(c));
    g_comms.erase(it);
}

int render_multi_impl(PrtScene* const* scenes, int n, const PrtCamera* cam, const PrtRenderParams* p, float* rgb_f32) {
    std::vector<int> devs(n);
    for (int r = 0; r < n; ++r) {
        if (!scenes[r]) return fail(PRT_E_INVALID, "prt_render_multi: null scene");
        if (scenes[r]->device < 0) return fail(PRT_E_NO_DEVICE, "prt_render_multi: a scene is not uploaded to a HIP device (no CPU path exists)");
        for (int q = 0; q < r; ++q)
            if (scenes[q] == scenes[r]) return fail(PRT_E_INVALID, "prt_render_multi: the same scene handle twice (one handle per tile share)");
        devs[r] = scenes[r]->device;
    }
    bool all_same = true, all_distinct = true;
    for (int r = 0; r < n; ++r)
        for (int q = 0; q < r; ++q) {
            if (devs[q] == devs[r]) all_distinct = false;
            else all_same = false;
        }
    if (n > 1 && !all_same && !all_distinct)
        return fail(PRT_E_INVALID, "prt_render_multi: scenes must sit on pairwise different devices (RCCL reduce) or all on one device");
    const size_t npx = (size_t)cam->width * cam->height * 3;
    for (int r = 0; r < n; ++r) {
        PrtScene* s = scenes[r];
        PRT_HIP(hipSetDevice(s->device));
// ... 754 lines not shown
```

pooraytracer_amd/csrc/prt_device.h:

```cpp
#pragma once
#include <hip/hip_runtime.h>
#include <stdint.h>

#include "prt_types.h"
#include "prt_light_pick.h"
#include "prt_wave.h"

#define PRT_DEV __device__ __forceinline__
typedef prt_real real;
#define PRT_F32 (sizeof(prt_real) == 4)
#define RL(x) ((real)(x))
template <typename R> struct real4_of;
template <> struct real4_of<double> { typedef double4 type; };
template <> struct real4_of<float> { typedef float4 type; };
typedef real4_of<real>::type real4;
#define PRT_NOCUR ((int32_t)0x80000000)
#ifndef PRT_BOX_PK
#define PRT_BOX_PK 1
#endif
#ifndef PRT_LEAF_BATCH
#define PRT_LEAF_BATCH 32
#endif
#ifndef PRT_INNER_MIN
#define PRT_INNER_MIN 12
#endif

struct d3 {
    real x, y, z;
};
struct d2 {
    real x, y;
};
PRT_DEV d3 mk3(real x, real y, real z) { return d3{x, y, z}; }
PRT_DEV d3 ld3(const real* p) { return d3{p[0], p[1], p[2]}; }
PRT_DEV d3 operator+(d3 a, d3 b) { return {a.x + b.x, a.y + b.y, a.z + b.z}; }
PRT_DEV d3 operator-(d3 a, d3 b) { return {a.x - b.x, a.y - b.y, a.z - b.z}; }
PRT_DEV d3 operator-(d3 a) { return {-a.x, -a.y, -a.z}; }
PRT_DEV d3 operator*(d3 a, d3 b) { return {a.x * b.x, a.y * b.y, a.z * b.z}; }
PRT_DEV d3 operator*(d3 a, real s) { return {a.x * s, a.y * s, a.z * s}; }
PRT_DEV d3 operator*(real s, d3 a) { return {s * a.x, s * a.y, s * a.z}; }
PRT_DEV d3 operator/(d3 a, real s);
PRT_DEV real dot(d3 a, d3 b) { return a.x * b.x + a.y * b.y + a.z * b.z; }
PRT_DEV d3 cross(d3 x, d3 y) { return {x.y * y.z - y.y * x.z, x.z * y.x - y.z * x.x, x.x * y.y - y.x * x.y}; }
PRT_DEV double fast_rsqrt(double x) {
    const double y = __builtin_amdgcn_rsq(x);
    const double g = x * y, h = 0.5 * y;
    const double r = fma(-h, g, 0.5);
    const double h1 = fma(h, r, h), g1 = fma(g, r, g);
    const double e = fma(-h1, g1, 0.5);
    return 2.0 * fma(h1, e, h1);
}
PRT_DEV double fast_sqrt(double x) {
    const double y = __builtin_amdgcn_rsq(x);
    const double g = x * y, h = 0.5 * y;
    const double r = fma(-h, g, 0.5);
    const double g1 = fma(g, r, g), h1 = fma(h, r, h);
    const double d = fma(-g1, g1, x);
    const double s = fma(d, h1, g1);
    return x == 0.0 ? 0.0 : s;
}
PRT_DEV double fast_rcp(double b) {
    double r = __builtin_amdgcn_rcp(b);
    r = fma(fma(-b, r, 1.0), r, r);
    r = fma(fma(-b, r, 1.0), r, r);
    return r;
}
PRT_DEV double fast_div(double a, double b) {
    const double r = fast_rcp(b);
    const double q = a * r;
    return fma(fma(-b, q, a), r, q);
}
PRT_DEV float fast_rsqrt(float x) { return __builtin_amdgcn_rsqf(x); }
PRT_DEV float fast_sqrt(float x) { return __builtin_amdgcn_sqrtf(x); }
PRT_DEV float fast_rcp(float b) { return __builtin_amdgcn_rcpf(b); }
PRT_DEV float fast_div(float a, float b) { return a * __builtin_amdgcn_rcpf(b); }
PRT_DEV double ieee_sqrt(double x) { return sqrt(x); }
PRT_DEV float ieee_sqrt(float x) { return __builtin_amdgcn_sqrtf(x); }
PRT_DEV double ieee_div(double a, double b) { return a / b; }
PRT_DEV float ieee_div(float a, float b) { return a * __builtin_amdgcn_rcpf(b); }
PRT_DEV d3 operator/(d3 a, real s) {
    const real r = fast_rcp(s);
    return {a.x * r, a.y * r, a.z * r};
}
PRT_DEV real length(d3 v) { return fast_sqrt(dot(v, v)); }
PRT_DEV d3 normalize(d3 v) { return v * fast_rsqrt(dot(v, v)); }
PRT_DEV d3 normalize_len(d3 v, real& len) {
    const real q = dot(v, v);
    const real inv = fast_rsqrt(q);
    len = q * inv;
    return v * inv;
}

#define PRT_PI RL(3.14159265358979323846)
#define PRT_INV_PI RL(0.31830988618379067154)
#define PRT_INV_2PI RL(0.15915494309189533577)
#define PRT_PI_OVER_2 RL(1.57079632679489661923)
#define PRT_PI_OVER_4 RL(0.78539816339744830961)
#define PRT_INF RL(__builtin_huge_val())

PRT_DEV uint64_t mix64(uint64_t z) {
    z ^= z >> 30;
    z *= 0xBF58476D1CE4E5B9ULL;
    z ^= z >> 27;
    z *= 0x94D049BB133111EBULL;
    z ^= z >> 31;
    return z;
}
PRT_DEV uint64_t seed_key(uint64_t seed) { return mix64(seed + 0x9E3779B97F4A7C15ULL); }
struct Rng {
    uint64_t s;
    PRT_DEV void seed_keyed(uint64_t key, uint64_t pixel, uint64_t sample) {
        s = mix64(((uint64_t)((uint32_t)(key >> 32) ^ (uint32_t)(pixel + 1)) << 32) | ((uint32_t)key ^ (uint32_t)(sample + 1)));
        if (s == 0) s = 0x9E3779B97F4A7C15ULL;
    }
    PRT_DEV void seed(uint64_t seed, uint64_t pixel, uint64_t sample) { seed_keyed(seed_key(seed), pixel, sample); }
    PRT_DEV real next() {
        uint32_t s0 = (uint32_t)s, s1 = (uint32_t)(s >> 32);
        const uint32_t r = s0 * 0x9E3779BBu;
        s1 ^= s0;
        s0 = __builtin_amdgcn_alignbit(s0, s0, 6) ^ s1 ^ (s1 << 9);
        s1 = __builtin_amdgcn_alignbit(s1, s1, 19);
        s = ((uint64_t)s1 << 32) | s0;
        if (PRT_F32) return (real)(r >> 8) * RL(5.9604644775390625e-8);
        return (real)(r >> 1) * (RL(1.0) / RL(2147483648.0));
    }
};

struct HitInfo {
    real t;
    real alpha, beta;
    int32_t tri;
};

struct WorkCount {
    uint32_t nodes, tris;
    uint32_t tris_full;
    uint32_t inner_rounds, leaf_rounds;
};
template <bool COUNT>
__device__ __forceinline__ void flush_trace_counts(DCounters* ctr, int lane, unsigned long long* rays_counter, uint32_t nrays, const WorkCount& wc) {
    const unsigned long long a = wave_sum((unsigned long long)nrays);
    const unsigned long long b = wave_sum((unsigned long long)wc.nodes);
    const unsigned long long c = wave_sum((unsigned long long)wc.tris);
    const unsigned long long f = wave_sum((unsigned long long)wc.tris_full);
    if (lane == 0) {
        atomicAdd(rays_counter, a);
        if (COUNT) {
            atomicAdd(&ctr->node_fetches, b);
            atomicAdd(&ctr->tri_tests, c);
            atomicAdd(&ctr->tri_full, f);
        }
    }
}

template <bool PAD>
PRT_DEV const DTri* tri_at(const DScene& S, uint32_t i) {
    return reinterpret_cast<const DTri*>(reinterpret_cast<const char*>(S.tris) + (size_t)i * (PAD ? PRT_TRI_PAD_STRIDE(real) : (uint32_t)sizeof(DTri)));
}

PRT_DEV bool tri_test(const DTri* __restrict__ T, d3 o, d3 d, real tmin, real tmax, real& t_out, real& a_out,
                      real& b_out, const real4* pre = nullptr, uint32_t* n_full = nullptr) {
    const real4* q = reinterpret_cast<const real4*>(T);
    real4 q0 = pre ? *pre : q[0], q1 = q[1];
    d3 n = mk3(q0.x, q0.y, q0.z);
    real denom = dot(n, d);
    if (fabs(denom) < RL(1e-8)) return false;
    real t = ieee_div(q0.w - dot(n, o), denom);
    if (!(tmin <= t && t <= tmax)) return false;
    if (n_full) ++*n_full;
    const real4 q2 = q[2];
    const d3 p = o + d * t;
    const real alpha = (p.x * q1.x + p.y * q1.y + p.z * q1.z) - q1.w;
    const real beta = (p.x * q2.x + p.y * q2.y + p.z * q2.z) - q2.w;
    if (alpha != alpha || beta != beta) return false;
    if ((alpha < 0) || (beta < 0) || (alpha + beta > 1)) return false;
    t_out = t;
    a_out = alpha;
    b_out = beta;
    return true;
}

PRT_DEV real dot_yxz(real ax, real ay, real az, real bx, real by, real bz) { return fma(az, bz, fma(ax, bx, ay * by)); }
PRT_DEV bool tri_test_ord(const DTri* __restrict__ T, d3 o, d3 d, real tmin, real tmax, real& t_out, real& a_out,
                          real& b_out, const real4& q0, uint32_t* n_full) {
    const real4* q = reinterpret_cast<const real4*>(T);
    real4 q1 = q[1];
    real denom = dot_yxz(q0.x, q0.y, q0.z, d.x, d.y, d.z);
    if (fabs(denom) < RL(1e-8)) return false;
    real t = ieee_div(q0.w - dot_yxz(q0.x, q0.y, q0.z, o.x, o.y, o.z), denom);
    if (!(tmin <= t && t <= tmax)) return false;
    if (n_full) ++*n_full;
    const real4 q2 = q[2];
    const d3 p = mk3(fma(d.x, t, o.x), fma(d.y, t, o.y), fma(d.z, t, o.z));
    const real alpha = dot_yxz(p.x, p.y, p.z, q1.x, q1.y, q1.z) - q1.w;
    const real beta = dot_yxz(p.x, p.y, p.z, q2.x, q2.y, q2.z) - q2.w;
    if (!(alpha >= 0 && beta >= 0 && alpha + beta <= 1)) return false;
    t_out = t;
    a_out = alpha;
    b_out = beta;
    return true;
}

PRT_DEV unsigned long long lane_mask(bool p) { return __builtin_amdgcn_ballot_w64(p); }

PRT_DEV float f32_up(real x) {
    const float f = (float)x;
    return f + fabsf(f) * 2.4e-7f;
}
PRT_DEV float f32_down(real x) {
    const float f = (float)x;
    return f - fabsf(f) * 2.4e-7f;
}

struct SlabAxis {
    float idq, c_lo, c_hi;
    uint32_t rot;
};
PRT_DEV SlabAxis slab_axis(real o, real d, float E, float g0, float gs) {
    SlabAxis a;
    const float df = (float)d;
    float id = __builtin_amdgcn_rcpf(df);
    if (!(fabsf(id) <= 1e28f)) id = copysignf(1e28f, df);
    const float r = (float)((real)g0 - o);
    const float c = r * id;
    const float pad = fmaf(E, fabsf(id), fabsf(c)) * 9.5367432e-7f;
    a.idq = gs * id;
    a.c_lo = c - pad;
    a.c_hi = c + pad;
    a.rot = id >= 0.f ? 0u : 16u;
    return a;
}

template <bool PAD, bool PK = false>
struct Trav {
    d3 o, d;
    real tmin;
    HitInfo hit;
    SlabAxis ax, ay, az;
    float tminf, tbestf;
    int32_t cur;
    int32_t sp;
    bool active;

    PRT_DEV void init(const DScene& S, d3 o_, d3 d_, real tmin_, real tmax_) {
        o = o_;
        d = d_;
        start(S, tmin_, tmax_);
    }
    PRT_DEV void start(const DScene& S, real tmin_, real tmax_) {
        tmin = tmin_;
        ax = slab_axis(o.x, d.x, S.slab_scale, S.grid_origin[0], S.grid_step[0]);
        ay = slab_axis(o.y, d.y, S.slab_scale, S.grid_origin[1], S.grid_step[1]);
        az = slab_axis(o.z, d.z, S.slab_scale, S.grid_origin[2], S.grid_step[2]);
        tminf = f32_down(tmin_);
        tbestf = f32_up(tmax_);
        hit.t = tmax_;
        hit.tri = -1;
        sp = 0;
        cur = 0;
        active = S.n_tris != 0;
    }

    PRT_DEV void box4(uint32_t x, uint32_t y, uint32_t z, float& n, float& f) const {
        x = __builtin_amdgcn_alignbit(x, x, ax.rot);
        y = __builtin_amdgcn_alignbit(y, y, ay.rot);
        z = __builtin_amdgcn_alignbit(z, z, az.rot);
        float nx, fx, ny, fy, nz, fz;
        if (PK) {
        typedef float f2_ __attribute__((ext_vector_type(2)));
        const f2_ tx = __builtin_elementwise_fma(f2_{(float)(x & 0xffffu), (float)(x >> 16)}, f2_{ax.idq, ax.idq}, f2_{ax.c_lo, ax.c_hi});
        const f2_ ty = __builtin_elementwise_fma(f2_{(float)(y & 0xffffu), (float)(y >> 16)}, f2_{ay.idq, ay.idq}, f2_{ay.c_lo, ay.c_hi});
        const f2_ tz = __builtin_elementwise_fma(f2_{(float)(z & 0xffffu), (float)(z >> 16)}, f2_{az.idq, az.idq}, f2_{az.c_lo, az.c_hi});
        nx = tx.x, fx = tx.y, ny = ty.x, fy = ty.y, nz = tz.x, fz = tz.y;
        } else {
        nx = fmaf((float)(x & 0xffffu), ax.idq, ax.c_lo), fx = fmaf((float)(x >> 16), ax.idq, ax.c_hi);
        ny = fmaf((float)(y & 0xffffu), ay.idq, ay.c_lo), fy = fmaf((float)(y >> 16), ay.idq, ay.c_hi);
        nz = fmaf((float)(z & 0xffffu), az.idq, az.c_lo), fz = fmaf((float)(z >> 16), az.idq, az.c_hi);
        }
        n = fmaxf(fmaxf(fmaxf(nx, ny), nz), tminf);
        f = fminf(fminf(fminf(fx, fy), fz), tbestf);
    }
    template <bool COUNT>
    PRT_DEV void inner_step(const DScene& S, uint32_t* stk, WorkCount& wc) {
        const uint4* np = reinterpret_cast<const uint4*>(reinterpret_cast<const char*>(S.nodes) + ((uint32_t)cur << 6));
        const uint4 bx = np[0], by = np[1], bz = np[2], rf = np[3];
        if (COUNT) wc.nodes++;
        float n0, f0, n1, f1, n2, f2, n3, f3;
        box4(bx.x, by.x, bz.x, n0, f0);
        box4(bx.y, by.y, bz.y, n1, f1);
        box4(bx.z, by.z, bz.z, n2, f2);
        box4(bx.w, by.w, bz.w, n3, f3);
        uint32_t k0 = n0 <= f0 ? __float_as_uint(n0) : 0xffffffffu;
        uint32_t k1 = n1 <= f1 ? __float_as_uint(n1) : 0xffffffffu;
        uint32_t k2 = (n2 <= f2 && rf.z != 0x80000000u) ? __float_as_uint(n2) : 0xffffffffu;
        uint32_t k3 = (n3 <= f3 && rf.w != 0x80000000u) ? __float_as_uint(n3) : 0xffffffffu;
        uint32_t r0 = rf.x, r1 = rf.y, r2 = rf.z, r3 = rf.w;
#define PRT_CE(ka, ra, kb, rb)                  \
    {                                           \
        const bool sw_ = kb < ka;               \
        const uint32_t tk_ = sw_ ? kb : ka;     \
        kb = sw_ ? ka : kb;                     \
        ka = tk_;                               \
        const uint32_t tr_ = sw_ ? rb : ra;     \
        rb = sw_ ? ra : rb;                     \
        ra = tr_;                               \
    }
        PRT_CE(k0, r0, k1, r1)
        PRT_CE(k2, r2, k3, r3)
        PRT_CE(k0, r0, k2, r2)
        PRT_CE(k1, r1, k3, r3)
        PRT_CE(k1, r1, k2, r2)
#undef PRT_CE
        const bool h1 = k1 != 0xffffffffu, h2 = k2 != 0xffffffffu, h3 = k3 != 0xffffffffu;
        sp += (int32_t)h1 + (int32_t)h2 + (int32_t)h3;
        uint32_t* const top = stk + sp * 64;
        if (h3) top[-3 * 64] = r3;
        if (h2) top[-2 * 64] = r2;
        if (h1) top[-1 * 64] = r1;
        if (k0 != 0xffffffffu) {
            cur = (int32_t)r0;
        } else if (sp == 0) {
            cur = PRT_NOCUR;
        } else {
            sp--;
            cur = (int32_t)stk[sp * 64];
        }
        if (cur == PRT_NOCUR) active = false;
    }

    template <bool COUNT>
    PRT_DEV bool test_leaf(const DScene& S, int32_t ref, WorkCount& wc, real tmin_use, bool any_hit) {
        const uint32_t enc = ~(uint32_t)ref;
        const uint32_t first = enc >> 3, cnt = (enc & 7u) + 1u;
        bool stop = false;
        real4 q0n = *reinterpret_cast<const real4*>(tri_at<PAD>(S, first));
        for (uint32_t i = 0; i < cnt; ++i) {
            real t, al, be;
            if (COUNT) wc.tris++;
            const real4 q0c = q0n;
            if (i + 1 < cnt) q0n = *reinterpret_cast<const real4*>(tri_at<PAD>(S, first + i + 1));
            if (tri_test(tri_at<PAD>(S, first + i), o, d, tmin_use, hit.t, t, al, be, &q0c, COUNT ? &wc.tris_full : nullptr)) {
                hit.t = t;
                if (!any_hit) {
                    hit.alpha = al;
                    hit.beta = be;
                }
                hit.tri = (int32_t)(first + i);
                tbestf = f32_up(t);
                if (any_hit) stop = true;
            }
        }
        return stop;
    }

    template <bool COUNT>
    PRT_DEV bool test_leaf_pp(const DScene& S, int32_t ref, WorkCount& wc, real tmin_use, bool any_hit) {
        const uint32_t enc = ~(uint32_t)ref;
        const uint32_t first = enc >> 3, cnt = (enc & 7u) + 1u;
        constexpr uint32_t STRIDE = PAD ? PRT_TRI_PAD_STRIDE(real) : (uint32_t)sizeof(DTri);
        const char* rec = reinterpret_cast<const char*>(tri_at<PAD>(S, first));
        bool stop = false;
        uint32_t i = 0;
        auto test = [&](const real4& q0) {
            real t, al, be;
            if (COUNT) wc.tris++;
            if (tri_test_ord(reinterpret_cast<const DTri*>(rec), o, d, tmin_use, hit.t, t, al, be, q0, COUNT ? &wc.tris_full : nullptr)) {
                hit.t = t;
                if (!any_hit) {
                    hit.alpha = al;
                    hit.beta = be;
                }
                hit.tri = (int32_t)(first + i);
                tbestf = f32_up(t);
                if (any_hit) stop = true;
            }
        };
        real4 qa = *reinterpret_cast<const real4*>(rec), qb;
        for (;;) {
            if (i + 1 < cnt) qb = *reinterpret_cast<const real4*>(rec + STRIDE);
            test(qa);
            if (++i == cnt) break;
            rec += STRIDE;
            if (i + 1 < cnt) qa = *reinterpret_cast<const real4*>(rec + STRIDE);
            test(qb);
            if (++i == cnt) break;
            rec += STRIDE;
        }
        return stop;
    }

    template <bool COUNT, bool PP = false>
    PRT_DEV void leaf_step(const DScene& S, uint32_t* stk, WorkCount& wc, real tmin_use, bool any_hit) {
        bool stop = false;
        if (cur < 0 && cur != PRT_NOCUR) {
            if constexpr (PP) stop = test_leaf_pp<COUNT>(S, cur, wc, tmin_use, any_hit);
            else stop = test_leaf<COUNT>(S, cur, wc, tmin_use, any_hit);
            cur = PRT_NOCUR;
        }
        if (stop) {
            active = false;
        } else if (cur == PRT_NOCUR) {
            if (sp == 0) active = false;
            else {
                sp--;
                cur = (int32_t)stk[sp * 64];
            }
        }
    }

    template <bool COUNT>
    PRT_DEV void round(const DScene& S, uint32_t* stk, WorkCount& wc, int leaf_batch, int inner_min, real tmin_use,
                       bool any_hit) {
        if (COUNT && __ballot(active && cur >= 0) != 0ULL) wc.inner_rounds++;
        if (active && cur >= 0) inner_step<COUNT>(S, stk, wc);
        const bool parked = active && cur < 0;
        const bool has_leaf = active && cur < 0 && cur != PRT_NOCUR;
        const int n_parked = __popcll(__ballot(parked));
        const int n_inner = __popcll(__ballot(active && cur >= 0));
        if (n_parked >= leaf_batch || n_inner <= inner_min) {
            if (COUNT && __ballot(has_leaf) != 0ULL) wc.leaf_rounds++;
            if (has_leaf) leaf_step<COUNT>(S, stk, wc, tmin_use, any_hit);
        }
    }
};

PRT_DEV int wave_count(bool p) { return __popcll(__ballot(p)); }

#define PRT_TEX_QUAD_REALS 16
template <bool EXTRA, bool NARROW = false>
PRT_DEV d3 tex_value(const DScene& S, int ti, real u, real v) {
    const DTexture tx = S.textures[ti];
    if (!tx.has_data) return mk3(RL(0.), RL(1.), RL(1.));
    u = fmin(fmax(u, RL(0.0)), RL(1.0));
    v = fmin(fmax(v, RL(0.0)), RL(1.0));
    real x = u * (tx.width - RL(1.));
    real y = (RL(1.) - v) * (tx.height - RL(1.));
    int x0 = (int)x, y0 = (int)y;
    real fx = x - x0, fy = y - y0;
    d3 c00, c10, c01, c11;
    if (!EXTRA || !S.tex_compact) {
        const real4* q = reinterpret_cast<const real4*>(S.texels_lin + tx.offset + (size_t)(y0 * tx.width + x0) * PRT_TEX_QUAD_REALS);
        if (NARROW) {
            const real4 r0 = q[0], r1 = q[1];
            const d3 top = mk3(r0.x, r0.y, r0.z) * (1 - fx) + mk3(r0.w, r1.x, r1.y) * fx;
            __builtin_amdgcn_sched_barrier(0);
            const real4 r2 = q[2];
            const d3 bot = mk3(r1.z, r1.w, r2.x) * (1 - fx) + mk3(r2.y, r2.z, r2.w) * fx;
            return top * (1 - fy) + bot * fy;
        }
        const real4 q0 = q[0], q1 = q[1], q2 = q[2];
        c00 = mk3(q0.x, q0.y, q0.z), c10 = mk3(q0.w, q1.x, q1.y);
        c01 = mk3(q1.z, q1.w, q2.x), c11 = mk3(q2.y, q2.z, q2.w);
    } else {
        const int x1 = min(x0 + 1, tx.width - 1), y1 = min(y0 + 1, tx.height - 1);
        const real* base = S.texels_lin + tx.offset;
        if (NARROW) {
            const d3 top = ld3(base + ((size_t)y0 * tx.width + x0) * 3) * (1 - fx) + ld3(base + ((size_t)y0 * tx.width + x1) * 3) * fx;
            __builtin_amdgcn_sched_barrier(0);
            const d3 bot = ld3(base + ((size_t)y1 * tx.width + x0) * 3) * (1 - fx) + ld3(base + ((size_t)y1 * tx.width + x1) * 3) * fx;
            return top * (1 - fy) + bot * fy;
        }
        c00 = ld3(base + ((size_t)y0 * tx.width + x0) * 3), c10 = ld3(base + ((size_t)y0 * tx.width + x1) * 3);
        c01 = ld3(base + ((size_t)y1 * tx.width + x0) * 3), c11 = ld3(base + ((size_t)y1 * tx.width + x1) * 3);
    }
    d3 c0 = c00 * (1 - fx) + c10 * fx;
    d3 c1 = c01 * (1 - fx) + c11 * fx;
    return c0 * (1 - fy) + c1 * fy;
}

PRT_DEV double fma_ks(double a, double b, double k) {
#if defined(__HIP_DEVICE_COMPILE__)
    double r;
    asm("v_fma_f64 %0, %1, %2, %3" : "=v"(r) : "v"(a), "v"(b), "s"(k));
    return r;
#else
    return __builtin_fma(a, b, k);
#endif
}
PRT_DEV float fma_ks(float a, float b, float k) { return __builtin_fmaf(a, b, k); }
PRT_DEV double fma_sk(double a, double k, double c) {
#if defined(__HIP_DEVICE_COMPILE__)
    double r;
    asm("v_fma_f64 %0, %1, %2, %3" : "=v"(r) : "v"(a), "s"(k), "v"(c));
    return r;
#else
    return __builtin_fma(a, k, c);
// ... 398 lines not shown
```

pooraytracer_amd/csrc/prt_host.h:

```cpp
#pragma once
#include <stdint.h>

#include <string>
#include <vector>

#include "../../include/prt.h"
#include "prt_types.h"

namespace prt {

struct HostTri {
    double v[3][3];
    double e0[3], e1[3];
    double uv[3][2];
    double normal[3], tangent[3];
    double area, D, w[3];
    double lo[3], hi[3];
    int32_t material, prim;
};

struct BuiltBVH {
    std::vector<DNode> nodes;
    std::vector<DNode> nodes_shallow;
    int stack_need = 0;
    std::vector<uint32_t> order;
    uint32_t depth = 0;
    float coord_scale = 1.0f;
    float grid_origin[3] = {0, 0, 0}, grid_step[3] = {1, 1, 1};
    struct BinNode {
        float lo[2][3], hi[2][3];
        int32_t ref[2];
    };
    bool keep_binary = false;
    std::vector<BinNode> binary;
};

struct PrimBox {
    float lo[3], hi[3];
};
void prim_boxes(const std::vector<HostTri>& tris, std::vector<PrimBox>& out, float origin[3]);
void quant_grid(const float root_lo[3], const float root_hi[3], bool empty, float origin[3], float step[3]);

struct DeviceBVH {
    DNode* d_nodes = nullptr;
    uint32_t* d_order = nullptr;
    uint32_t n_nodes = 0, depth = 0;
    float coord_scale = 1.0f;
    float grid_origin[3] = {0, 0, 0}, grid_step[3] = {1, 1, 1};
    double ms_sort = 0, ms_tree = 0, ms_split = 0, ms_total = 0;
};

struct LightTree {
    std::vector<DLightNode> nodes;
    std::vector<DLightTri> tris;
    int32_t root = -1;
    double area = 0.0;
    std::vector<uint32_t> tab;
    uint32_t n_tables = 0;
    std::vector<DLightNode> full_nodes;
    int32_t full_root = -1;
};
struct LightTablePlan {
    std::vector<uint32_t> tab;
    std::vector<int32_t> node;
    std::vector<double> area;
    std::vector<DLightNode> top;
    int32_t root = -1;
};
bool plan_light_tables(const LightTree& lt, LightTablePlan& plan);
void apply_light_tables(LightTree& lt, const LightTablePlan& plan, const std::vector<uint32_t>& tab);
int32_t light_pick(const LightTree& lt, float p);
int32_t light_pick_full_tree(const LightTree& lt, float p);

void setup_triangles(const PrtSceneDesc& d, std::vector<HostTri>& out);
void update_triangles(const double* vertices, const double* normals, std::vector<HostTri>& tris);
void update_triangles_listed(const int32_t* prims, size_t n, const double* vertices, const double* normals, std::vector<HostTri>& tris);
void setup_materials(const PrtSceneDesc& d, std::vector<DMaterial>& out);
bool build_bvh(const std::vector<HostTri>& tris, BuiltBVH& out, std::string* err);
bool node_count_ok(size_t n_nodes, std::string* err);
bool validate_nodes(const DNode* nodes, size_t n_nodes, size_t n_tris, std::string* err);
int tree_stack_need(const DNode* nodes, size_t n_nodes);
bool build_bvh_device(const PrimBox* h_boxes, const float box_origin[3], size_t n, DeviceBVH& out, std::string* err);
void build_light_tree(const PrtSceneDesc& d, const std::vector<HostTri>& tris, const std::vector<DMaterial>& mats,
                      LightTree& out, bool with_tables = true);
void setup_camera(const PrtCamera& c, DCamera& out);

inline uint64_t seed_key(uint64_t seed) {
    uint64_t z = seed + 0x9E3779B97F4A7C15ULL;
    z ^= z >> 30;
    z *= 0xBF58476D1CE4E5B9ULL;
    z ^= z >> 27;
    z *= 0x94D049BB133111EBULL;
    z ^= z >> 31;
    return z;
}

}
```

pooraytracer_amd/csrc/prt_kernels.hip:

```cpp
#include <hip/hip_runtime.h>

#include <type_traits>

#include "../../include/prt.h"
#include "prt_device.h"
#include "prt_launch.h"

#ifndef PRT_F32_TU
#define PRT_F32_TU 0
#endif
#if PRT_F32_TU
#define PRT_NS prt32
#else
#define PRT_NS prt
#endif
#define PRT_DYN_STACK PRT_F32_TU

#ifndef PRT_RENDER_WAVES
#define PRT_RENDER_WAVES 2
#endif
#ifndef PRT_RENDER_WAVES_LEAN
#define PRT_RENDER_WAVES_LEAN 3
#endif
#ifndef PRT_RENDER_WAVES_TEX
// ... 185 lines not shown
        q[11] = make_double2(0.0, 0.0);
        const d3 a = feature_albedo<PRT_FEAT_ALL | PRT_FEAT_EXTRA | PRT_FEAT_NARROW>(S, m, uv);
        q[7] = make_double2((double)uv.y, (double)a.x);
        q[8] = make_double2((double)a.y, (double)a.z);
    } else {
        const double2 z = make_double2(0.0, 0.0);
        q[0] = make_double2((double)PRT_INF, 0.0);
        q[1] = make_double2(0.0, __longlong_as_double(0x00000000ffffffffLL));
        for (int k = 2; k < 12; ++k) q[k] = z;
        q[10] = make_double2(0.0, __longlong_as_double(-1LL));
    }
}

template <bool COUNT, bool PAD>
__global__ __launch_bounds__(PRT_BLOCK, PRT_K1S_WAVES) void k_trace_surface(DScene S, const PrtRay* __restrict__ rays, size_t n,
                                                                            PrtSurface* __restrict__ out, DCounters* ctr,
                                                                            const uint32_t* __restrict__ perm) {
    __shared__ uint32_t s_stack[PRT_BLOCK / 64][PRT_STACK_DEPTH][64];
    const int lane = threadIdx.x & 63, wave = threadIdx.x >> 6;
    uint32_t* stk = &s_stack[wave][0][lane];
    WorkCount wc{0, 0, 0, 0, 0};
    uint32_t nrays = 0;
    Trav<PAD> tr;
    tr.init(S, mk3(0, 0, 0), mk3(0, 0, 1), RL(0.0), RL(0.0));
    tr.hit.alpha = tr.hit.beta = RL(0.0);
    tr.active = false;
    bool have = false;
    size_t my = 0;
    WavePool<PRT_K1_CHUNK> pool;
    for (;;) {
        if (!tr.active && have) {
            surface_record<PAD>(S, tr.o, tr.d, tr.hit, out + my);
            have = false;
        }
        {
            const unsigned long long need = __ballot(!tr.active);
            if (pool.wants(need)) {
                pool.refill(need, lane, n, &ctr->next_item);
                if (!pool.exhausted && !tr.active) {
                    const unsigned long long idx = pool.index(need, lane);
                    if (idx < pool.end) {
                        const size_t ri = perm ? (size_t)perm[idx] : (size_t)idx;
                        const double4* rp = reinterpret_cast<const double4*>(rays + ri);
                        const double4 r0 = rp[0], r1 = rp[1];
                        tr.init(S, mk3((real)r0.x, (real)r0.y, (real)r0.z), mk3((real)r1.x, (real)r1.y, (real)r1.z), (real)r0.w, (real)r1.w);
                        my = ri;
                        have = true;
                        nrays++;
                    }
                }
                pool.advance(need);
            }
        }
        if (__ballot(tr.active || have) == 0ULL && pool.exhausted) break;
        do {
            tr.template round<COUNT>(S, stk, wc, PRT_LEAF_BATCH, PRT_INNER_MIN, tr.tmin, false);
        } while (wave_count(tr.active) > PRT_K1_KEEP);
    }
    flush_trace_counts<COUNT>(ctr, lane, &ctr->rays_closest, nrays, wc);
}

template <int PARK_STRIDE>
PRT_DEV void park_real(uint32_t* base, int word, real v) {
    if (PRT_F32) {
        base[word * PARK_STRIDE] = __float_as_uint((float)v);
    } else {
        const unsigned long long b = (unsigned long long)__double_as_longlong((double)v);
        base[word * PARK_STRIDE] = (uint32_t)b;
        base[(word + 1) * PARK_STRIDE] = (uint32_t)(b >> 32);
    }
}
template <int PARK_STRIDE>
PRT_DEV real unpark_real(const uint32_t* base, int word) {
    if (PRT_F32) return (real)__uint_as_float(base[word * PARK_STRIDE]);
    return (real)__longlong_as_double((long long)(((unsigned long long)base[(word + 1) * PARK_STRIDE] << 32) | base[word * PARK_STRIDE]));
}
#define PRT_RW ((int)(sizeof(real) / 4))
#define PARK_T 0
#define PARK_TRI PRT_RW
#define PARK_DIR (PRT_RW + 1)
#define PARK_DIR_GLOBAL(feat) (((feat) & PRT_FEAT_TEX) != 0)
#define PARK_AB_AT(feat) (PARK_DIR_GLOBAL(feat) ? PRT_RW + 1 : 4 * PRT_RW + 1)
#define PARK_WORDS(feat) (((feat) & PRT_FEAT_TEX) ? 3 * PRT_RW + 1 : 4 * PRT_RW + 1)

PRT_DEV void load_ray(const void* ray_list, uint32_t i, d3& o, d3& d) {
    const PrtRay* r = static_cast<const PrtRay*>(ray_list) + i;
    o = mk3((real)r->o[0], (real)r->o[1], (real)r->o[2]);
    d = mk3((real)r->d[0], (real)r->d[1], (real)r->d[2]);
}

template <typename R>
struct RenderArgsT {
    DSceneT<R> S;
    DCameraT<R> C;
    DRenderParamsT<R> P;
    double* partial;
    DCounters* ctr;
};
typedef RenderArgsT<real> RenderArgs;
typedef const RenderArgs __attribute__((address_space(4)))* ColdRenderArgs;
PRT_DEV ColdRenderArgs cold_args() {
    ColdRenderArgs q = (ColdRenderArgs)__builtin_amdgcn_kernarg_segment_ptr();
    asm volatile("" : "+s"(q));
    return q;
}

template <bool COUNT, int FEAT, bool LLDS, bool PAD>
__global__ __launch_bounds__(PRT_BLOCK, render_waves(FEAT)) void k_render(RenderArgs A) {
    const DScene& S = A.S;
    const DRenderParams& P = A.P;
    DCounters* const ctr = A.ctr;
    constexpr bool RAYS = (FEAT & PRT_FEAT_RAYS) != 0;
    constexpr bool PLAIN = (FEAT & PRT_FEAT_PLAIN) != 0;
    static_assert(!PLAIN || (!COUNT && !RAYS && LLDS), "PLAIN: production frame kernels with LDS tables only");
#define JITTER (!PLAIN && P.jitter)
#define FROM_LIST (!PLAIN && P.scramble == PRT_ITEMS_FROM_LIST)
#define SAMPLE_LIGHTS (PLAIN || P.sample_lights)
#define HAS_LIGHTS (PLAIN || S.n_lights > 0)
#define LTRI_LDS (PLAIN ? 1 : P.ltri_lds)
    __shared__ uint32_t s_qoff[PRT_BLOCK / 64];
    __shared__ unsigned long long s_rays[PRT_BLOCK / 64];
    __shared__ real s_center[4];
    constexpr int NPARK = PRT_BLOCK;
    __shared__ uint32_t s_park[PARK_WORDS(FEAT)][NPARK];
#define park (&s_park[0][threadIdx.x])
    const int lane = threadIdx.x & 63, wave = threadIdx.x >> 6;
    extern __shared__ __align__(16) unsigned char s_dyn_all[];
#if PRT_DYN_STACK
    uint32_t* stk = reinterpret_cast<uint32_t*>(s_dyn_all) + (size_t)(wave * P.stack_depth) * 64 + lane;
    unsigned char* s_dyn = s_dyn_all + (size_t)(PRT_BLOCK / 64) * P.stack_depth * 64 * sizeof(uint32_t);
#else
    __shared__ uint32_t s_stack[PRT_BLOCK / 64][PRT_STACK_DEPTH][64];
    uint32_t* stk = &s_stack[wave][0][lane];
    unsigned char* s_dyn = s_dyn_all;
#endif
    if (lane == 0) {
        s_qoff[wave] = 0;
        s_rays[wave] = 0ULL;
    }
    if (threadIdx.x < 3) s_center[threadIdx.x] = A.C.center[threadIdx.x];
    if (!LLDS) __syncthreads();
    const DLightNode* lds_lights = reinterpret_cast<const DLightNode*>(s_dyn);
    const DMaterial* lds_mats = reinterpret_cast<const DMaterial*>(s_dyn + (size_t)P.light_lds * sizeof(DLightNode));
    const DLightTri* lds_ltris = reinterpret_cast<const DLightTri*>(s_dyn + (size_t)P.light_lds * sizeof(DLightNode) + (size_t)P.mat_lds * sizeof(DMaterial));
    if (LLDS) {
        uint4* dst = reinterpret_cast<uint4*>(s_dyn);
        const uint4* src = reinterpret_cast<const uint4*>(S.light_nodes);
        for (int i = threadIdx.x; i < P.light_lds; i += PRT_BLOCK) dst[i] = src[i];
        dst += P.light_lds;
        src = reinterpret_cast<const uint4*>(S.materials);
        const int nm = P.mat_lds * (int)(sizeof(DMaterial) / 16);
        for (int i = threadIdx.x; i < nm; i += PRT_BLOCK) dst[i] = src[i];
        dst += nm;
        src = reinterpret_cast<const uint4*>(S.light_tris);
        const int nl = P.ltri_lds * (int)(sizeof(DLightTri) / 16);
        for (int i = threadIdx.x; i < nl; i += PRT_BLOCK) dst[i] = src[i];
        __syncthreads();
    }
#define MATERIAL(i) (LLDS ? lds_mats[(i)] : S.materials[(i)])
    d3 pst_[2];
#define PST_LD(k) (pst_[(k) / 3])
#define PST_ST(k, v) (pst_[(k) / 3] = (v))
#define S_ACC 0
#define S_BETA 3
#define ADD_RADIANCE(x) PST_ST(S_ACC, PST_LD(S_ACC) + (PST_LD(S_BETA) * (x)) * inv_spp)
#define TRACING (COUNT && P.scramble == PRT_ITEMS_FROM_LIST && ctr->trace != nullptr)
#define TRACE_VERTEX(prim_)                                                     \
    do {                                                                        \
        if (TRACING) {                                                          \
            const int v_ = P.max_depth - depth;                                 \
            if (v_ < PRT_TRACE_VERTS) {                                         \
                int32_t* tw_ = ctr->trace + (size_t)item * PRT_TRACE_WORDS;     \
                tw_[0] = v_ + 1;                                                \
                tw_[1 + 2 * v_] = (prim_);                                      \
                tw_[2 + 2 * v_] = 0;                                            \
            }                                                                   \
        }                                                                       \
    } while (0)
#define TRACE_FLAG_AT(v_, bit_)                                                 \
    do {                                                                        \
        if (TRACING) {                                                          \
            if ((v_) < PRT_TRACE_VERTS) ctr->trace[(size_t)item * PRT_TRACE_WORDS + 2 + 2 * (v_)] |= (bit_); \
        }                                                                       \
    } while (0)
#define TRACE_FLAG(bit_)                                                        \
    do {                                                                        \
        if (TRACING) {                                                          \
            const int v_ = P.max_depth - depth;                                 \
            if (v_ < PRT_TRACE_VERTS) ctr->trace[(size_t)item * PRT_TRACE_WORDS + 2 + 2 * v_] |= (bit_); \
        }                                                                       \
    } while (0)

    WorkCount wc{0, 0, 0, 0, 0};
    uint32_t n_refills = 0;

    int state = ST_FETCH;
    uint32_t item = 0;
    int px = 0, py = 0, s = 0, s_end = 0, depth = 0;
    uint32_t pixel = 0;
    bool first = true, prev_skip = false;
    PST_ST(S_ACC, mk3(0, 0, 0));
    PST_ST(S_BETA, mk3(1, 1, 1));
    d3 rd = mk3(0, 0, 1);
    int32_t sh_tri = -1;
    real ldist = 0;
    int32_t ltri = 0;
    constexpr bool ONE_PASS = PRT_ONE_PASS_VERTEX && !(FEAT & (PRT_FEAT_PHONG | PRT_FEAT_TEX));
    constexpr bool EVAL_FLAT = ONE_PASS && !(FEAT & PRT_FEAT_CT);
    constexpr bool TURN = ONE_PASS && PRT_SAMPLE_TURNOVER && !(PRT_F32 && !(FEAT & PRT_FEAT_CT));
    constexpr bool WAVE_DIET = ONE_PASS && !PRT_F32;
    d3 pending = mk3(0, 0, 0);
    d3 next_d = mk3(0, 0, 1);
    bool cont = false;
    int nee_v = 0;
    Rng rng;
    rng.s = 0;
    const real inv_spp = RL(1.0) / (real)P.spp;
    Trav<PAD, PRT_BOX_PK != 0> tr;
    tr.init(S, mk3(0, 0, 0), rd, RL(0.0), RL(0.0));
    tr.hit.alpha = tr.hit.beta = RL(0.0);
    tr.active = false;

#if PRT_K3_PROFILE
    unsigned long long prof_[6] = {0, 0, 0, 0, 0, 0}, prof_t_ = __builtin_readcyclecounter();
#endif
#define END_OF_SAMPLE(next) do {                                                                                                                                          \
        s++;                                                                                                                                                              \
        if (s < s_end) state = (next);                                                                                                                                     \
        else {                                                                                                                                                            \
            const d3 acc = PST_LD(S_ACC);                                         \
            double* o = cold_args()->partial + (size_t)item * 3;                                                                                                          \
            o[0] = (double)acc.x;                                                                    \
            o[1] = (double)acc.y;                                                                                                                                         \
            o[2] = (double)acc.z;                                                                                                                                         \
            state = ST_FETCH;                                                                                                                                             \
        }                                                                                                                                                                 \
    } while (0)
#define NEW_SAMPLE(parked) do {                                                                                                                                           \
                                                                                                                            \
        rng.seed_keyed(P.seed_key, (uint64_t)pixel, (uint64_t)s);                                                                                                         \
        if (!RAYS && JITTER) {                                                                                                                                            \
                                                           \
                                                                                                                      \
            const ColdRenderArgs q = cold_args();                                                                                                                         \
            const int W = q->C.width;                                                                                                                                     \
            const int jy = (int)(pixel / (uint32_t)W), jx = (int)(pixel - (uint32_t)jy * (uint32_t)W);                                                                    \
            const real fy = (real)jy + (rng.next() - RL(0.5));                                                                                                            \
            const real fx = (real)jx + (rng.next() - RL(0.5));                                                                                                            \
            const d3 ps = mk3(q->C.pixel00[0], q->C.pixel00[1], q->C.pixel00[2]) + fx * mk3(q->C.du[0], q->C.du[1], q->C.du[2]) +                                         \
                          fy * mk3(q->C.dv[0], q->C.dv[1], q->C.dv[2]);                                                                                                   \
            tr.o = mk3(q->C.center[0], q->C.center[1], q->C.center[2]);                                                                                                   \
            tr.d = ps - tr.o;                                                                                                                                             \
            state = ST_CLOSEST;                                                                                                                                           \
        } else {                                                                                                                                                          \
                                                        \
                                                 \
                                                        \
            if (RAYS) {                                                                          \
                load_ray(ctr->ray_list, (uint32_t)px, tr.o, tr.d);                                                                                                        \
            } else if (PARK_DIR_GLOBAL(FEAT)) {                                               \
                tr.o = mk3(s_center[0], s_center[1], s_center[2]);                                                                                                        \
                const ColdRenderArgs q = cold_args();                                                                                                                     \
                const d3 ps = mk3(q->C.pixel00[0], q->C.pixel00[1], q->C.pixel00[2]) + (real)px * mk3(q->C.du[0], q->C.du[1], q->C.du[2]) +                               \
                              (real)py * mk3(q->C.dv[0], q->C.dv[1], q->C.dv[2]);                                                                                         \
                tr.d = ps - tr.o;                                                                                                                                         \
            } else {                                                                                                                                                      \
                tr.o = mk3(s_center[0], s_center[1], s_center[2]);                                                                                                        \
                tr.d = mk3(unpark_real<NPARK>(park, PARK_DIR), unpark_real<NPARK>(park, PARK_DIR + PRT_RW), unpark_real<NPARK>(park, PARK_DIR + 2 * PRT_RW));             \
            }                                                                                                                                                             \
            tr.hit.t = unpark_real<NPARK>(park, PARK_T);                                                                                                                  \
            tr.hit.tri = (int32_t)park[PARK_TRI * NPARK];                                                                                                                 \
            if (FEAT & PRT_FEAT_TEX) {                                                                                                                                    \
                tr.hit.alpha = unpark_real<NPARK>(park, PARK_AB_AT(FEAT));                                                                                                \
                tr.hit.beta = unpark_real<NPARK>(park, PARK_AB_AT(FEAT) + PRT_RW);                                                                                        \
            }                                                                                                                                                             \
            state = (parked);                                                                                                                                             \
        }                                                                                                                                                                 \
        PST_ST(S_BETA, mk3(1, 1, 1));                                                                                                                                     \
        depth = P.max_depth;                                                                                                                                              \
        first = true;                                                                                                                                                     \
        prev_skip = false;                                                                                                                                                \
    } while (0)
    for (;;) {
        if (COUNT) n_refills++;
        PROF_MARK(0);
        int started = 0;
        if (!tr.active) {
            bool end_sample = false, do_scatter = false;
            bool nee = false;
            bool have_fr = false;
            d3 fr_seen = mk3(0, 0, 0);
            if (state == ST_PRIMARY) {
                bool flat = false;
// ... 283 lines not shown
                    const uint32_t oi = item - chunk * ipc;
                    const int W = q->C.width;
                    bool valid;
                    if (RAYS) {
                        px = (int)oi;
                        valid = true;
                    } else if (FROM_LIST) {
                        const int32_t pix = ctr->pixel_list[oi];
                        py = pix / W;
                        px = pix - py * W;
                        valid = true;
                        if (COUNT && ctr->trace != nullptr) ctr->trace[(size_t)item * PRT_TRACE_WORDS] = 0;
                    } else {
                        valid = tile_pixel(P.scramble, ipc, q->P.tile, q->P.tiles_x, q->P.n_tiles, q->P.rank, q->P.nranks, W, q->C.height, oi, px, py);
                    }
                    if (valid) {
                        s = q->P.chunk_begin[chunk];
                        s_end = q->P.chunk_begin[chunk + 1];
                        if (RAYS) {
                            const uint32_t* keys = ctr->key_list;
                            pixel = keys ? keys[oi] : oi;
                        } else {
                            pixel = (uint32_t)(py * W + px);
                        }
                        PST_ST(S_ACC, mk3(0, 0, 0));
                        if (s >= s_end) {
                            double* o = q->partial + (size_t)item * 3;
                            o[0] = o[1] = o[2] = 0.0;
                        } else if (RAYS) {
                            load_ray(ctr->ray_list, oi, tr.o, tr.d);
                            state = ST_PRIMARY;
                        } else if (JITTER) {
                            state = TURN ? ST_CACHED : ST_NEW_SAMPLE;
                        } else {
                            const d3 ps = mk3(q->C.pixel00[0], q->C.pixel00[1], q->C.pixel00[2]) + (real)px * mk3(q->C.du[0], q->C.du[1], q->C.du[2]) +
                                          (real)py * mk3(q->C.dv[0], q->C.dv[1], q->C.dv[2]);
                            tr.o = mk3(q->C.center[0], q->C.center[1], q->C.center[2]);
                            tr.d = ps - tr.o;
                            if (!PARK_DIR_GLOBAL(FEAT)) {
                                park_real<NPARK>(park, PARK_DIR, tr.d.x);
                                park_real<NPARK>(park, PARK_DIR + PRT_RW, tr.d.y);
                                park_real<NPARK>(park, PARK_DIR + 2 * PRT_RW, tr.d.z);
                            }
                            state = ST_PRIMARY;
                        }
                    }
                }
            }
            if (!TURN && state == ST_NEW_SAMPLE) NEW_SAMPLE(ST_CACHED);
            PROF_MARK(3);
            if (state == ST_CLOSEST || state == ST_SHADOW || state == ST_PRIMARY) {
                const bool sh_ray = state == ST_SHADOW;
                started = sh_ray ? 2 : 1;
                if (WAVE_DIET && take_next) tr.d = next_d;
                if (COUNT && ctr->ray_dump != nullptr) {
                    const unsigned long long k = atomicAdd(&ctr->ray_dump_n, 1ULL);
                    if (k < ctr->ray_dump_cap) {
                        PrtRay r;
                        r.o[0] = (double)tr.o.x; r.o[1] = (double)tr.o.y; r.o[2] = (double)tr.o.z;
                        r.d[0] = (double)tr.d.x; r.d[1] = (double)tr.d.y; r.d[2] = (double)tr.d.z;
                        r.tmin = sh_ray ? 0.001 : 0.0001;
                        r.tmax = sh_ray ? (double)(ldist - RL(0.001)) : __builtin_huge_val();
                        static_cast<PrtRay*>(ctr->ray_dump)[k] = r;
                    }
                }
                tr.start(S, sh_ray ? RL(0.001) : RL(0.0001), sh_ray ? ldist - RL(0.001) : PRT_INF);
            }
        }
        PROF_MARK(4);
        {
            const unsigned long long nc = (unsigned long long)__popcll(__ballot(started == 1)), ns = (unsigned long long)__popcll(__ballot(started == 2));
            if (lane == 0) atomicAdd(&s_rays[wave], nc | (ns << 32));
        }
        if (__ballot(state != ST_DONE) == 0ULL) break;
        if (wave_count(state == ST_CACHED) >= P.cached_min) continue;

        if constexpr (WAVE_DIET) {
            bool sh = state == ST_SHADOW;
            unsigned long long m_chain = lane_mask(sh && cont);
            unsigned long long m_act;
            if (!tr.active) tr.cur = PRT_NOCUR;
            do {
                if (COUNT && lane_mask(tr.cur >= 0) != 0ULL) wc.inner_rounds++;
                if (tr.cur >= 0) tr.template inner_step<COUNT>(S, stk, wc);
                const unsigned long long m_inner = lane_mask(tr.cur >= 0);
                const unsigned long long m_parked = lane_mask((uint32_t)tr.cur > (uint32_t)PRT_NOCUR);
                m_act = m_inner | m_parked;
                if (__popcll(m_parked) >= P.leaf_batch || __popcll(m_inner) <= P.inner_min) {
                    if (COUNT && m_parked != 0ULL) wc.leaf_rounds++;
                    if ((uint32_t)tr.cur > (uint32_t)PRT_NOCUR) tr.template leaf_step<COUNT, !COUNT>(S, stk, wc, sh ? RL(0.001) : RL(0.0001), sh);
                    m_act = lane_mask(tr.cur != PRT_NOCUR);
                }
                const unsigned long long m_fin = m_chain & ~m_act;
                if (__popcll(m_fin) >= P.chain_min) {
                    PROF_MARK(0);
                    if (tr.cur == PRT_NOCUR && sh && cont) {
                        if (tr.hit.tri < 0) {
                            PST_ST(S_ACC, PST_LD(S_ACC) + pending);
                            TRACE_FLAG_AT(nee_v, PRT_TRACE_VISIBLE);
                        }
                        tr.d = next_d;
                        state = ST_CLOSEST;
                        sh = false;
                        if (COUNT && ctr->ray_dump != nullptr) {
                            const unsigned long long k = atomicAdd(&ctr->ray_dump_n, 1ULL);
                            if (k < ctr->ray_dump_cap) {
                                PrtRay r;
                                r.o[0] = (double)tr.o.x; r.o[1] = (double)tr.o.y; r.o[2] = (double)tr.o.z;
                                r.d[0] = (double)tr.d.x; r.d[1] = (double)tr.d.y; r.d[2] = (double)tr.d.z;
                                r.tmin = 0.0001;
                                r.tmax = __builtin_huge_val();
                                static_cast<PrtRay*>(ctr->ray_dump)[k] = r;
                            }
                        }
                        tr.start(S, RL(0.0001), PRT_INF);
                        if (!tr.active) tr.cur = PRT_NOCUR;
                    }
                    if (lane == 0) atomicAdd(&s_rays[wave], (unsigned long long)__popcll(m_fin));
                    m_chain &= m_act;
                    m_act = lane_mask(tr.cur != PRT_NOCUR);
                    PROF_MARK(5);
                }
            } while (__popcll(m_act) > P.keep);
            tr.active = tr.cur != PRT_NOCUR;
        } else
        do {
            tr.template round<COUNT>(S, stk, wc, P.leaf_batch, P.inner_min, state == ST_SHADOW ? RL(0.001) : RL(0.0001), state == ST_SHADOW);
            if (ONE_PASS) {
                const bool fin = !tr.active && state == ST_SHADOW && cont;
                const int n_fin = wave_count(fin);
                if (n_fin >= P.chain_min) {
                    PROF_MARK(0);
                    if (fin) {
                        if (tr.hit.tri < 0) {
                            PST_ST(S_ACC, PST_LD(S_ACC) + pending);
                            TRACE_FLAG_AT(nee_v, PRT_TRACE_VISIBLE);
                        }
                        tr.d = next_d;
                        state = ST_CLOSEST;
                        if (COUNT && ctr->ray_dump != nullptr) {
                            const unsigned long long k = atomicAdd(&ctr->ray_dump_n, 1ULL);
                            if (k < ctr->ray_dump_cap) {
                                PrtRay r;
                                r.o[0] = (double)tr.o.x; r.o[1] = (double)tr.o.y; r.o[2] = (double)tr.o.z;
                                r.d[0] = (double)tr.d.x; r.d[1] = (double)tr.d.y; r.d[2] = (double)tr.d.z;
                                r.tmin = 0.0001;
                                r.tmax = __builtin_huge_val();
                                static_cast<PrtRay*>(ctr->ray_dump)[k] = r;
                            }
                        }
                        tr.start(S, RL(0.0001), PRT_INF);
                    }
                    if (lane == 0) atomicAdd(&s_rays[wave], (unsigned long long)n_fin);
                    PROF_MARK(5);
                }
            }
        } while (wave_count(tr.active) > P.keep);
    }

    unsigned long long d = wave_sum((unsigned long long)wc.nodes);
    unsigned long long e = wave_sum((unsigned long long)wc.tris);
    unsigned long long f = wave_sum((unsigned long long)wc.tris_full);
    if (lane == 0) {
        const unsigned long long rays = s_rays[wave];
        atomicAdd(&ctr->rays_closest, rays & 0xffffffffULL);
        atomicAdd(&ctr->rays_shadow, rays >> 32);
        if (COUNT) {
            atomicAdd(&ctr->tri_full, f);
#if PRT_K3_PROFILE
            atomicAdd(&ctr->node_fetches, prof_[5]);
            atomicAdd(&ctr->tri_tests, prof_[0]);
            atomicAdd(&ctr->inner_rounds, prof_[1]);
            atomicAdd(&ctr->leaf_rounds, prof_[2]);
// ... 281 lines not shown
    const d3 p00 = mk3(C.pixel00[0], C.pixel00[1], C.pixel00[2]), du = mk3(C.du[0], C.du[1], C.du[2]), dv = mk3(C.dv[0], C.dv[1], C.dv[2]);
    d3 a_sum = mk3(0, 0, 0), n_sum = mk3(0, 0, 0);
    double z_sum = 0.0;
    int n_hit = 0;
    int32_t prim0 = -1;
    WorkCount wc{0, 0, 0, 0, 0};
    Trav<PAD> tr;
    const int traced = jitter ? spp : 1;
    for (int s = 0; s < traced; ++s) {
        real fx = (real)px, fy = (real)py;
        if (jitter) {
            Rng rng;
            rng.seed_keyed(seed_key, (uint64_t)pix, (uint64_t)s);
            fy = fy + (rng.next() - RL(0.5));
            fx = fx + (rng.next() - RL(0.5));
        }
        const d3 ps = p00 + fx * du + fy * dv;
        tr.init(S, center, ps - center, RL(0.0001), PRT_INF);
        tr.hit.alpha = tr.hit.beta = RL(0.0);
        if (!valid) tr.active = false;
        while (__ballot(tr.active) != 0ULL) tr.template round<false>(S, stk, wc, PRT_LEAF_BATCH, PRT_INNER_MIN, RL(0.0001), false);
        if (!valid) continue;
        if (s == 0) prim0 = tr.hit.tri >= 0 ? S.shade[tr.hit.tri].prim : -1;
        if (tr.hit.tri < 0) {
            a_sum = a_sum + mk3(1, 1, 1);
            continue;
        }
        const DTriShade* sh = S.shade + tr.hit.tri;
        const DMaterial& m = S.materials[sh->material];
        const d3 gn = ld3(tri_at<PAD>(S, (uint32_t)tr.hit.tri)->n);
        const d3 fn = face_normal(tr.d, gn);
        const d2 uv = hit_uv(sh, tr.hit.alpha, tr.hit.beta);
        const d3 a = feature_albedo<PRT_FEAT_ALL | PRT_FEAT_EXTRA>(S, m, uv);
        a_sum = a_sum + a;
        n_sum = n_sum + fn;
        z_sum += (double)tr.hit.t * sqrt((double)dot(tr.d, tr.d));
        n_hit++;
    }
    if (!valid) return;
    const real nt = (real)traced;
    if (albedo) {
        albedo[(size_t)pix * 3] = (float)(a_sum.x / nt);
        albedo[(size_t)pix * 3 + 1] = (float)(a_sum.y / nt);
        albedo[(size_t)pix * 3 + 2] = (float)(a_sum.z / nt);
    }
    if (normal) {
        normal[(size_t)pix * 3] = (float)(n_sum.x / nt);
        normal[(size_t)pix * 3 + 1] = (float)(n_sum.y / nt);
        normal[(size_t)pix * 3 + 2] = (float)(n_sum.z / nt);
    }
    if (depth) depth[pix] = n_hit ? (float)(z_sum / (double)n_hit) : __builtin_huge_valf();
    if (prim) prim[pix] = prim0;
}

__global__ void k_add_f32(float* __restrict__ dst, const float* __restrict__ src, size_t n) {
    const size_t i = (size_t)blockIdx.x * blockDim.x + threadIdx.x;
    if (i < n) dst[i] += src[i];
}

#endif

}

namespace PRT_NS {

int render_permutation(int feat) {
    feat &= ~(PRT_FEAT_RAYS | PRT_FEAT_PLAIN);
    if (feat == 0 || feat == PRT_FEAT_TEX || feat == PRT_FEAT_PHONG || feat == PRT_FEAT_CT) return feat;
    return PRT_FEAT_ALL;
}

int render_lds_budget(int feat, int stack_depth) {
    int blocks = render_waves(render_permutation(feat));
    if (PRT_F32_TU && stack_depth <= 32) blocks = PRT_F32_WAVES > 4 && stack_depth <= 24 ? 5 : 4;
    const int perm = render_permutation(feat);
    return ((160 * 1024 / blocks - (int)sizeof(uint32_t) * (stack_depth + PARK_WORDS(perm)) * PRT_BLOCK - 256) / 512) * 512;
}
size_t render_table_bytes(int light_lds, int mat_lds, int ltri_lds) {
    return (size_t)light_lds * sizeof(DLightNode) + (size_t)mat_lds * sizeof(DMaterial) + (size_t)ltri_lds * sizeof(DLightTri);
}

typedef void (*RenderKernel)(RenderArgs);
constexpr bool plain_permutation(int perm) { return !PRT_F32_TU && perm != PRT_FEAT_TEX; }
bool render_plain(int feat, bool count, bool rays, int n_lights, int ltri_lds, int jitter, int scramble, int sample_lights) {
    return plain_permutation(render_permutation(feat)) && !count && !rays && n_lights > 0 && ltri_lds > 0 && !jitter &&
           scramble != PRT_ITEMS_FROM_LIST && sample_lights;
}
template <int FEAT, bool PAD>
static RenderKernel render_kernel_feat(bool count, bool llds, bool extra, bool rays, bool plain) {
    constexpr int X = FEAT | PRT_FEAT_EXTRA;
    if constexpr (plain_permutation(FEAT)) {
        if (plain) return extra ? k_render<false, X | PRT_FEAT_PLAIN, true, PAD> : k_render<false, FEAT | PRT_FEAT_PLAIN, true, PAD>;
    }
    if (rays) return llds ? k_render<false, X | PRT_FEAT_RAYS, true, PAD> : k_render<false, X | PRT_FEAT_RAYS, false, PAD>;
    if (count) return llds ? k_render<true, X, true, PAD> : k_render<true, X, false, PAD>;
    if (extra) return llds ? k_render<false, X, true, PAD> : k_render<false, X, false, PAD>;
    return llds ? k_render<false, FEAT, true, PAD> : k_render<false, FEAT, false, PAD>;
}
template <bool PAD>
static RenderKernel render_kernel_pad(bool count, int feat, bool llds, bool extra) {
    const bool rays = (feat & PRT_FEAT_RAYS) != 0;
    const bool plain = (feat & PRT_FEAT_PLAIN) != 0 && llds && !count && !rays;
    switch (render_permutation(feat)) {
    case 0: return render_kernel_feat<0, PAD>(count, llds, extra, rays, plain);
    case PRT_FEAT_TEX: return render_kernel_feat<PRT_FEAT_TEX, PAD>(count, llds, extra, rays, plain);
    case PRT_FEAT_PHONG: return render_kernel_feat<PRT_FEAT_PHONG, PAD>(count, llds, extra, rays, plain);
    case PRT_FEAT_CT: return render_kernel_feat<PRT_FEAT_CT, PAD>(count, llds, extra, rays, plain);
    default: return render_kernel_feat<PRT_FEAT_ALL, PAD>(count, llds, extra, rays, plain);
    }
}
static RenderKernel render_kernel(bool count, int feat, bool llds, bool pad, bool extra) {
    return pad ? render_kernel_pad<true>(count, feat, llds, extra) : render_kernel_pad<false>(count, feat, llds, extra);
}

static size_t stack_bytes(int stack_depth) { return PRT_DYN_STACK ? (size_t)PRT_BLOCK * stack_depth * sizeof(uint32_t) : 0; }

int render_blocks_per_cu(bool count, int feat, size_t table_bytes, int stack_depth, bool pad, bool extra, bool rays, bool plain) {
    int nb = 0;
    if (rays) feat |= PRT_FEAT_RAYS;
    if (plain) feat |= PRT_FEAT_PLAIN;
    hipError_t e = hipOccupancyMaxActiveBlocksPerMultiprocessor(&nb, render_kernel(count, feat, table_bytes != 0, pad, extra), PRT_BLOCK,
                                                                table_bytes + stack_bytes(stack_depth));
    if (e != hipSuccess || nb < 1) nb = 1;
    return nb;
}

hipError_t launch_trace(const DScene& S, const PrtRay* d_rays, size_t n, void* d_out, DCounters* d_ctr, bool count, int mode,
                        int n_cu, hipStream_t st, const uint32_t* d_perm) {
    if (n == 0) return hipGetLastError();
    size_t want = (n + PRT_BLOCK - 1) / PRT_BLOCK;
    const size_t per_cu = std::max<size_t>(1, (160u * 1024u) / (sizeof(uint32_t) * PRT_STACK_DEPTH * PRT_BLOCK));
    unsigned grid = (unsigned)std::min<size_t>(want, (size_t)n_cu * per_cu);
    const bool pad = S.tri_stride == PRT_TRI_PAD_STRIDE(real) && sizeof(DTri) != PRT_TRI_PAD_STRIDE(real);
    const bool any_hit = mode == PRT_TRACE_ANY;
    const int pick = (count ? 4 : 0) | (pad ? 2 : 0) | (any_hit ? 1 : 0);
    auto go = [&](auto k, auto* out) {
        hipLaunchKernelGGL(k, dim3(grid), dim3(PRT_BLOCK), 0, st, S, d_rays, n, out, d_ctr, d_perm);
        return hipGetLastError();
    };
    PrtHit* hits = static_cast<PrtHit*>(d_out);
    uint8_t* bytes = static_cast<uint8_t*>(d_out);
    if (mode == PRT_TRACE_SURFACE) {
        PrtSurface* recs = static_cast<PrtSurface*>(d_out);
        switch (pick >> 1) {
        case 0: return go(k_trace_surface<false, false>, recs);
        case 1: return go(k_trace_surface<false, true>, recs);
        case 2: return go(k_trace_surface<true, false>, recs);
        default: return go(k_trace_surface<true, true>, recs);
        }
    }
    switch (pick) {
    case 0: return go(k_trace<false, false, false>, hits);
    case 1: return go(k_trace<false, false, true>, bytes);
    case 2: return go(k_trace<false, true, false>, hits);
    case 3: return go(k_trace<false, true, true>, bytes);
    case 4: return go(k_trace<true, false, false>, hits);
    case 5: return go(k_trace<true, false, true>, bytes);
    case 6: return go(k_trace<true, true, false>, hits);
    default: return go(k_trace<true, true, true>, bytes);
    }
}

void launch_render(const DScene& S, const DCamera& C, const DRenderParams& P, double* d_partial, DCounters* d_ctr,
                   bool count, int feat, unsigned grid, hipStream_t st, bool rays, bool plain) {
    static_assert(sizeof(DMaterial) % 16 == 0, "materials are staged in 16-byte pieces");
    const size_t tables = render_table_bytes(P.light_lds, P.mat_lds, P.ltri_lds);
    const size_t dyn_lds = tables + stack_bytes(P.stack_depth);
    const bool pad = S.tri_stride == PRT_TRI_PAD_STRIDE(real) && sizeof(DTri) != PRT_TRI_PAD_STRIDE(real);
    RenderArgs A;
// ... 148 lines not shown
```

pooraytracer_amd/csrc/prt_launch.h:

```cpp
#pragma once
#include <hip/hip_runtime.h>

#include <algorithm>
#include <string>

#include "../../include/prt.h"
#include "prt_types.h"

namespace prt {
int render_blocks_per_cu(bool count, int feat, size_t table_bytes, int stack_depth, bool pad, bool extra, bool rays, bool plain);
bool render_plain(int feat, bool count, bool rays, int n_lights, int ltri_lds, int jitter, int scramble, int sample_lights);
int render_permutation(int feat);
int render_lds_budget(int feat, int stack_depth);
size_t render_table_bytes(int light_lds, int mat_lds, int ltri_lds);
hipError_t launch_trace(const DSceneT<double>& S, const PrtRay* d_rays, size_t n, void* d_out, DCounters* d_ctr, bool count, int mode,
                        int n_cu, hipStream_t st, const uint32_t* d_perm);
size_t ray_sort_scratch_bytes(size_t n, std::string* err);
const uint32_t* ray_sort(const PrtRay* d_rays, size_t n, const float grid_origin[3], const float grid_step[3], void* scratch,
                         size_t scratch_bytes, hipStream_t st, std::string* err);
void launch_render(const DSceneT<double>& S, const DCameraT<double>& C, const DRenderParamsT<double>& P, double* d_partial,
                   DCounters* d_ctr, bool count, int feat, unsigned grid, hipStream_t st, bool rays, bool plain);
void launch_finalize(const DCameraT<double>& C, const DRenderParamsT<double>& P, const double* d_partial, double* d64, float* d32,
                     hipStream_t st);
void launch_finalize_rays(const DRenderParamsT<double>& P, const double* d_partial, double* d64, float* d32, hipStream_t st);
void launch_accumulate(const DCameraT<double>& C, const DRenderParamsT<double>& P, const double* d_partial, double* d_sum,
                       hipStream_t st);
void launch_resolve(const double* d_sum, size_t n, uint64_t samples, const uint32_t* d_counts, double* d64, float* d32,
                    uint8_t* d8, hipStream_t st);
uint32_t adapt_segments(uint64_t owned_items);
void launch_adapt_select(const DCameraT<double>& C, const DRenderParamsT<double>& P, const DAdaptRule& R, const double* d_sum,
                         const double* d_moment, const uint32_t* d_count, uint32_t* d_seg, int32_t* d_list, uint32_t* d_total,
                         hipStream_t st);
void launch_accumulate_list(const DRenderParamsT<double>& P, const double* d_partial, const int32_t* d_list, uint32_t batch,
                            uint32_t samples, double* d_sum, double* d_moment, uint32_t* d_count, hipStream_t st);
void launch_accum_variance(const double* d_sum, const double* d_moment, const uint32_t* d_count, size_t npx, uint32_t batch,
                           float* d_var, hipStream_t st);
void launch_sample_lights(const DSceneT<double>& S, const double* d_origins, size_t n, uint64_t seed, PrtLightSample* d_out,
                          hipStream_t st);
void launch_tonemap(const float* d_in, size_t n, uint8_t* d_out, hipStream_t st);
void launch_features(const DSceneT<double>& S, const DCameraT<double>& C, uint64_t seed_key, int jitter, int spp, float* albedo,
                     float* normal, float* depth, int32_t* prim, hipStream_t st);
void launch_add_f32(float* dst, const float* src, size_t n, hipStream_t st);
void launch_material_eval(const DSceneT<double>& S, int material, const double* wi, const double* wo, const double* uv, size_t n,
                          uint64_t seed, double* out, hipStream_t st);
void launch_material_scatter(const DSceneT<double>& S, int material, const double* rd, const double* normal, const double* tangent,
                             const double* uv, size_t n, uint64_t seed, double* wi_out, double* att_out, int32_t* ok_out,
                             hipStream_t st);
void launch_texture_value(const DSceneT<double>& S, int texture, const double* uv, size_t n, double* out, hipStream_t st);
size_t denoise_scratch_bytes(int w, int h);
void launch_denoise(int w, int h, const float* rgb, const float* albedo, const float* normal, const float* depth,
                    int iterations, int demod, const float sigma[4], void* scratch, float* out, hipStream_t st);
void launch_denoise_guided(int w, int h, const float* rgb, const float* var, const float* albedo, const float* normal,
                           const float* depth, int iterations, int demod, const float sigma[4], void* scratch, float* out,
                           float* out_var, hipStream_t st);
hipError_t launch_light_tables(const DLightTableBuild& A, hipStream_t st);
struct RefitCheck {
    double lo[3], hi[3];
    double scale;
    uint32_t flags;
    uint32_t pad_;
};
static_assert(sizeof(RefitCheck) == 64, "RefitCheck layout (the kernels write it, prt_api.cpp reads it back)");
size_t refit_scratch_bytes();
void launch_refit_check(const double* d_verts, uint32_t n, const DLightTriT<double>* d_ltris, uint32_t n_lights, void* d_scratch,
                        RefitCheck* d_out, hipStream_t st, const double* d_normals, double* d_gather_v, double* d_gather_n);
void launch_refit_tris(const double* d_verts, const double* d_normals, const uint32_t* d_order, uint32_t n, void* d_tris,
                       uint32_t tri_stride, DTriShadeT<double>* d_shade, float* d_tbox, const double origin[3], double delta,
                       hipStream_t st);
void launch_refit_parents(const DNode* d_nodes, uint32_t n_nodes, uint32_t* d_parent, hipStream_t st);
void launch_prim_boxes(const double* d_verts, uint32_t n, float* d_boxes, const double origin[3], double delta, hipStream_t st);
void launch_permute_shade(const DTriShadeT<double>* d_shade_old, const uint32_t* d_old_order, const uint32_t* d_new_order,
                          uint32_t n, uint32_t* d_inv, DTriShadeT<double>* d_shade_new, hipStream_t st);
hipError_t launch_refit_boxes(DNode* d_nodes, uint32_t n_nodes, const uint32_t* d_parent, uint32_t* d_cnt, const float* d_tbox,
                              uint32_t n_tris, const float step[3], hipStream_t st);
void launch_refit_sah(const DNode* d_nodes, uint32_t n_nodes, const float origin[3], const float step[3], void* d_scratch,
                      double* d_out, hipStream_t st);
struct PrimBox;
struct DeviceBVH;
bool build_bvh_device_boxes(const PrimBox* d_boxes, const float box_origin[3], size_t n, DeviceBVH& out, std::string* err,
                            hipStream_t st);
void launch_gather_tris(const DTriT<double>* tri_in, const DTriShadeT<double>* shade_in, const uint32_t* order, uint32_t n,
                        void* tri_out, uint32_t tri_out_stride, DTriShadeT<double>* shade_out, hipStream_t st);
inline hipError_t point_query_grid(const void* k, size_t n, size_t lds, int n_cu, bool plain, unsigned& grid) {
    if (lds > 64u * 1024u) {
        const hipError_t e = hipFuncSetAttribute(k, hipFuncAttributeMaxDynamicSharedMemorySize, (int)lds);
        if (e != hipSuccess) return e;
    }
    const size_t want = (n + PRT_BLOCK - 1) / PRT_BLOCK;
    const size_t per_cu = std::max<size_t>(1, std::min<size_t>(4, (160u * 1024u) / lds));
    grid = (unsigned)(plain ? want : std::min<size_t>(want, (size_t)std::max(n_cu, 1) * per_cu));
    return hipSuccess;
}
void launch_gather_corners(const double* d_verts, const uint32_t* d_order, uint32_t n, DTriCorners* d_out, hipStream_t st);
hipError_t launch_closest_point(const DSceneT<double>& S, const DTriCorners* d_corners, const PrtPointQuery* d_q, size_t n,
                                PrtClosestPoint* d_out, DCounters* d_ctr, bool count, int stack_depth, int n_cu, bool plain,
                                hipStream_t st);
struct DSignedTables;
hipError_t launch_signed_distance(const DSceneT<double>& S, const DTriCorners* d_corners, const DSignedTables& T, const PrtPointQuery* d_q,
                                  size_t n, PrtSignedDistance* d_out, DCounters* d_ctr, bool count, int stack_depth, int n_cu,
                                  hipStream_t st);
struct DSignedTables {
    const uint32_t* slot = nullptr;
    const uint32_t* v_start = nullptr;
    const uint32_t* v_list = nullptr;
    const uint32_t* e_start = nullptr;
    const uint32_t* e_list = nullptr;
    double* face = nullptr;
    double* normal = nullptr;
    uint32_t n_tris = 0, n_vertices = 0, n_edges = 0;
};
void launch_pseudonormals(const DTriCorners* d_corners, const DSignedTables& T, hipStream_t st);
struct alignas(64) DWindingMoment {
    double N[3];
    double c[3];
    double r;
    double A;
};
hipError_t launch_winding_moments(const DNode* d_nodes, uint32_t n_nodes, const uint32_t* d_parent, uint32_t* d_cnt,
                                  const DTriCorners* d_corners, uint32_t n_tris, DWindingMoment* d_mom, hipStream_t st);
hipError_t launch_winding_number(const DSceneT<double>& S, const DTriCorners* d_corners, const DWindingMoment* d_mom, const PrtPointQuery* d_q,
                                 size_t n, double beta, double* d_out, DCounters* d_ctr, bool count, int stack_depth, int n_cu,
                                 hipStream_t st);
hipError_t launch_multi_hit(const DSceneT<double>& S, const PrtRay* d_rays, const PrtHitCursor* d_after, size_t n, int k, PrtHit* d_out,
                            DCounters* d_ctr, bool count, int n_cu, hipStream_t st, const uint32_t* d_perm);
}

namespace prt32 {
int render_blocks_per_cu(bool count, int feat, size_t table_bytes, int stack_depth, bool pad, bool extra, bool rays, bool plain);
bool render_plain(int feat, bool count, bool rays, int n_lights, int ltri_lds, int jitter, int scramble, int sample_lights);
int render_permutation(int feat);
int render_lds_budget(int feat, int stack_depth);
size_t render_table_bytes(int light_lds, int mat_lds, int ltri_lds);
hipError_t launch_trace(const DSceneT<float>& S, const PrtRay* d_rays, size_t n, void* d_out, DCounters* d_ctr, bool count, int mode,
                        int n_cu, hipStream_t st, const uint32_t* d_perm);
void launch_render(const DSceneT<float>& S, const DCameraT<float>& C, const DRenderParamsT<float>& P, double* d_partial,
                   DCounters* d_ctr, bool count, int feat, unsigned grid, hipStream_t st, bool rays, bool plain);
void launch_convert_tris(const void* in, uint32_t in_stride, uint32_t n, void* out, uint32_t out_stride, hipStream_t st);
void launch_convert_shade(const DTriShadeT<double>* in, uint32_t n, DTriShadeT<float>* out, hipStream_t st);
void launch_convert_reals(const double* in, size_t n, float* out, hipStream_t st);
hipError_t launch_multi_hit(const DSceneT<float>& S, const PrtRay* d_rays, const PrtHitCursor* d_after, size_t n, int k, PrtHit* d_out,
                            DCounters* d_ctr, bool count, int n_cu, hipStream_t st, const uint32_t* d_perm);
}
```

pooraytracer_amd/csrc/scene_setup.cpp:

```cpp
#include <algorithm>
#include <cmath>
#include <cstring>
#include <limits>

#include "prt_host.h"

namespace prt {
namespace {

struct V {
    double x, y, z;
};
inline V sub(V a, V b) { return {a.x - b.x, a.y - b.y, a.z - b.z}; }
inline V add(V a, V b) { return {a.x + b.x, a.y + b.y, a.z + b.z}; }
inline V scale(V a, double s) { return {a.x * s, a.y * s, a.z * s}; }
inline double dot(V a, V b) { return a.x * b.x + a.y * b.y + a.z * b.z; }
inline V cross(V a, V b) { return {a.y * b.z - b.y * a.z, a.z * b.x - b.z * a.x, a.x * b.y - b.x * a.y}; }
inline V unit(V a) { return scale(a, 1.0 / std::sqrt(dot(a, a))); }
inline bool has_nan(V a) { return a.x != a.x || a.y != a.y || a.z != a.z; }
inline void store(double* p, V a) {
    p[0] = a.x;
    p[1] = a.y;
    p[2] = a.z;
}
// ... 6 lines not shown
        lo -= 0.0001 / 2.;
        hi += 0.0001 / 2.;
    }
}

}

static void setup_triangle_geometry(HostTri& T, const V p[3], const V vn[3]) {
    for (int k = 0; k < 3; ++k) store(T.v[k], p[k]);
    V e0 = sub(p[1], p[0]), e1 = sub(p[2], p[0]);
    V n = cross(e0, e1);
    V nn = unit(n);
    if (has_nan(nn)) {
        nn = unit(add(add(vn[0], vn[1]), vn[2]));
        if (has_nan(nn)) nn = V{0.0, 0.0, 1.0};
    }
    double du0 = T.uv[1][0] - T.uv[0][0], dv0 = T.uv[1][1] - T.uv[0][1];
    double du1 = T.uv[2][0] - T.uv[0][0], dv1 = T.uv[2][1] - T.uv[0][1];
    double f = 1.0 / (du0 * dv1 - du1 * dv0);
    V tg{f * (dv1 * e0.x - dv0 * e1.x), f * (dv1 * e0.y - dv0 * e1.y), f * (dv1 * e0.z - dv0 * e1.z)};
    tg = unit(tg);
    if (has_nan(tg)) {
        V helper = (std::fabs(nn.x) < (double)0.9f) ? V{1, 0, 0} : V{0, 1, 0};
        tg = unit(cross(nn, helper));
    }
    store(T.e0, e0);
    store(T.e1, e1);
    store(T.normal, nn);
    store(T.tangent, tg);
    T.area = std::sqrt(dot(n, n)) * 0.5;
    T.D = dot(nn, p[0]);
    double nn2 = dot(n, n);
    T.w[0] = n.x / nn2;
    T.w[1] = n.y / nn2;
    T.w[2] = n.z / nn2;
    for (int a = 0; a < 3; ++a) {
        double l0, h0, l1, h1;
        edge_interval(T.v[0][a], T.v[1][a], l0, h0);
        edge_interval(T.v[0][a], T.v[2][a], l1, h1);
        T.lo[a] = l0 <= l1 ? l0 : l1;
        T.hi[a] = h0 >= h1 ? h0 : h1;
    }
}

void setup_triangles(const PrtSceneDesc& d, std::vector<HostTri>& out) {
    out.resize(d.n_tris);
    for (uint32_t m = 0; m < d.n_meshes; ++m) {
        for (uint64_t t = d.mesh_first_tri[m]; t < d.mesh_first_tri[m + 1]; ++t) {
            HostTri& T = out[t];
            V p[3], vn[3];
            for (int k = 0; k < 3; ++k) {
                p[k] = load(d.vertices + t * 9 + k * 3);
                vn[k] = d.normals ? load(d.normals + t * 9 + k * 3) : V{0, 0, 0};
                T.uv[k][0] = d.texcoords ? d.texcoords[t * 6 + k * 2] : 0.0;
                T.uv[k][1] = d.texcoords ? d.texcoords[t * 6 + k * 2 + 1] : 0.0;
            }
            T.material = d.mesh_material[m];
            T.prim = (int32_t)t;
            setup_triangle_geometry(T, p, vn);
        }
    }
}

void update_triangles_listed(const int32_t* prims, size_t n, const double* vertices, const double* normals, std::vector<HostTri>& tris) {
    for (size_t i = 0; i < n; ++i) {
        V p[3], vn[3];
        for (int k = 0; k < 3; ++k) {
            p[k] = load(vertices + i * 9 + k * 3);
            vn[k] = normals ? load(normals + i * 9 + k * 3) : V{0, 0, 0};
        }
        setup_triangle_geometry(tris[(size_t)prims[i]], p, vn);
    }
}

void update_triangles(const double* vertices, const double* normals, std::vector<HostTri>& tris) {
    for (size_t t = 0; t < tris.size(); ++t) {
        V p[3], vn[3];
        for (int k = 0; k < 3; ++k) {
            p[k] = load(vertices + t * 9 + k * 3);
            vn[k] = normals ? load(normals + t * 9 + k * 3) : V{0, 0, 0};
        }
        setup_triangle_geometry(tris[t], p, vn);
    }
}

void setup_materials(const PrtSceneDesc& d, std::vector<DMaterial>& out) {
    out.resize(d.n_materials);
    for (uint32_t i = 0; i < d.n_materials; ++i) {
        const PrtMaterial& s = d.materials[i];
        DMaterial& m = out[i];
        std::memset(&m, 0, sizeof(m));
        m.type = s.type;
        m.texture = s.texture;
        for (int c = 0; c < 3; ++c) {
            m.kd[c] = s.kd[c];
            m.ks[c] = s.ks[c];
            m.eta[c] = s.eta[c];
            m.k[c] = s.k[c];
        }
        m.ns = s.ns;
        m.inv_ns1 = 1.0 / (s.ns + 1.0);
        m.spec_scale = (s.ns + 2.0) / (s.ns + 1.0);
        if (s.ns <= 9.) {
            m.pkd = 1.0;
            m.pks = 0.0;
        } else {
            m.pkd = 0.6;
            m.pks = 0.4;
        }
        m.alpha_x = s.alpha_x;
        m.alpha_y = s.alpha_y;
        m.has_emission = (s.type == PRT_MAT_DIFFUSE_LIGHT || s.type == PRT_MAT_DEBUG) ? 1 : 0;
        for (int c = 0; c < 3; ++c)
            m.emission[c] = s.type == PRT_MAT_DIFFUSE_LIGHT ? s.emission[c] : (s.type == PRT_MAT_DEBUG ? s.kd[c] : 0.0);
        m.skip_light_sampling =
            (s.type == PRT_MAT_MIRROR || s.type == PRT_MAT_EMPTY || (s.type == PRT_MAT_PHONG && s.ns > 1.)) ? 1 : 0;
    }
}

namespace {

struct Obj {
    int32_t tri;
    int32_t node;
};
struct TNode {
    double lo[3], hi[3];
    double area;
    Obj left, right;
    bool single;
};

struct RefBuilder {
    const std::vector<HostTri>& tris;
    std::vector<TNode> nodes;
    explicit RefBuilder(const std::vector<HostTri>& t) : tris(t) {}

    const double* lo(const Obj& o) const { return o.node < 0 ? tris[o.tri].lo : nodes[o.node].lo; }
    const double* hi(const Obj& o) const { return o.node < 0 ? tris[o.tri].hi : nodes[o.node].hi; }
    double area(const Obj& o) const { return o.node < 0 ? tris[o.tri].area : nodes[o.node].area; }

    int32_t build(std::vector<Obj>& objs, size_t start, size_t end) {
        TNode n;
        const double inf = std::numeric_limits<double>::infinity();
        for (int a = 0; a < 3; ++a) {
            n.lo[a] = inf;
            n.hi[a] = -inf;
        }
        for (size_t i = start; i < end; ++i)
            for (int a = 0; a < 3; ++a) {
                const double l = lo(objs[i])[a], h = hi(objs[i])[a];
                n.lo[a] = n.lo[a] <= l ? n.lo[a] : l;
                n.hi[a] = n.hi[a] >= h ? n.hi[a] : h;
            }
        const double lx = n.hi[0] - n.lo[0], ly = n.hi[1] - n.lo[1], lz = n.hi[2] - n.lo[2];
        const int axis = (lx > ly) ? (lx > lz ? 0 : 2) : (ly > lz ? 1 : 2);
        const size_t span = end - start;
        n.single = false;
        if (span == 1) {
            n.left = n.right = objs[start];
            n.area = area(objs[start]);
            n.single = true;
        } else if (span == 2) {
            n.left = objs[start];
            n.right = objs[start + 1];
            n.area = area(objs[start]) + area(objs[start + 1]);
// ... 363 lines not shown
```

Baseline: 14340 Mrays/s.

## Add bounded-scene fast fp64 division and biased LDS stack pushes in plain kernel

When every scene coordinate and the camera center lie below a fixed bound, the plain fp64 render kernel computes the triangle hit distance with a reciprocal-plus-Newton-refinement sequence instead of an IEEE division. The same kernel forms also merge the park and traversal stack into one shared struct. Stack pushes then go through a pre-biased LDS pointer with positive offsets, which should save address arithmetic in the inner BVH step. Host code tracks boundedness across scene creation, updates and refits and adds it as a condition for choosing the plain kernel. The risk is small accuracy differences in t and a more complex LDS layout.

```diff
diff --git a/pooraytracer_amd/csrc/prt_api.cpp b/pooraytracer_amd/csrc/prt_api.cpp
--- a/pooraytracer_amd/csrc/prt_api.cpp
+++ b/pooraytracer_amd/csrc/prt_api.cpp
@@ -161,6 +161,7 @@
     bool explicit_lights = false;
     bool device_bvh = false;
     uint64_t generation = 0;
+    bool bounded = true;
     PrtBvhInfo bvh_info{};
     int device = -1;
     int n_cu = 0;
@@ -446,10 +447,11 @@
 }
 
 template <typename R>
-static bool frame_plain(const PrtScene* s, const KernelConfig<R>& k, bool count, bool rays, int jitter, int scramble, int sample_lights) {
+static bool frame_plain(const PrtScene* s, const KernelConfig<R>& k, bool count, bool rays, int jitter, int scramble, int sample_lights, bool bounded) {
     const auto plain = std::is_same<R, double>::value ? prt::render_plain : prt32::render_plain;
-    return plain(s->feat, count, rays, k.d.n_lights, k.ltri_lds, jitter, scramble, sample_lights);
-}
+    return plain(s->feat, count, rays, k.d.n_lights, k.ltri_lds, jitter, scramble, sample_lights, bounded);
+}
+static bool frame_bounded(const PrtScene* s, const DCamera& C) { return s->bounded && prt::coords_bounded(C.center, 3); }
 static bool generic_forced() {
     const char* e = dev_env("PRT_TUNE_GENERIC");
     return e && std::atoi(e);
@@ -468,7 +470,7 @@
     auto blocks = [&](bool count, size_t tables, bool plain = false) { return blocks_per_cu(count, s->feat, tables, k.stack_depth, pad, extra, false, plain); };
     const size_t tables = table_bytes(k.light_lds, k.mat_lds, k.ltri_lds);
     k.blocks_per_cu[0] = blocks(false, tables);
-    k.blocks_per_cu[2] = frame_plain(s, k, false, false, 0, 0, 1) ? blocks(false, tables, true) : 0;
+    k.blocks_per_cu[2] = frame_plain(s, k, false, false, 0, 0, 1, true) ? blocks(false, tables, true) : 0;
     const int wanted = drop_tables && tables != 0 ? blocks(false, 0) : k.blocks_per_cu[0];
     if (k.blocks_per_cu[0] < wanted || (k.blocks_per_cu[2] && k.blocks_per_cu[2] < wanted)) {
         k.mat_lds = k.ltri_lds = k.light_lds = 0;
@@ -650,6 +652,7 @@
     if (!s) return fail(PRT_E_OOM, "prt_scene_create: out of host memory");
     try {
         prt::setup_triangles(*desc, s->tris);
+        s->bounded = prt::scene_bounded(s->tris);
         s->mesh_first.assign(desc->mesh_first_tri, desc->mesh_first_tri + (desc->n_meshes ? desc->n_meshes + 1 : 0));
         s->mesh_mat.assign(desc->mesh_material, desc->mesh_material + desc->n_meshes);
         s->explicit_lights = desc->light_meshes != nullptr;
@@ -1116,6 +1119,7 @@
     try {
         prt::update_triangles(vertices, normals, s->tris);
         s->host_stale = false;
+        s->bounded = prt::scene_bounded(s->tris);
         PrtSceneDesc d;
         light_desc(s, d);
         s->lights = prt::LightTree();
@@ -1303,6 +1307,7 @@
     float origin[3], step[3], root_hi[3];
     double origin_d[3], delta;
     bool lights_moved = false;
+    bool bounded = false;
 };
 
 static int refit_begin(PrtScene* s, const std::string& who, const double* d_verts, const double* d_normals, hipStream_t st,
@@ -1367,6 +1372,7 @@
         return fail(PRT_E_INVALID, who + ": a vertex of a light mesh moved; emitters stay in place under a refit (the light tree is not "
                                          "rebuilt) - use prt_scene_update_vertices");
     g.lights_moved = (c.flags & 2u) != 0;
+    g.bounded = prt::coords_bounded(c.lo, 3) && prt::coords_bounded(c.hi, 3);
     const double extent = std::max(1.0, std::max(c.hi[0] - c.lo[0], std::max(c.hi[1] - c.lo[1], c.hi[2] - c.lo[2])));
     g.delta = 1e-9 * extent + 256.0 * std::numeric_limits<double>::epsilon() * c.scale;
     for (int a = 0; a < 3; ++a) {
@@ -1556,8 +1562,9 @@
     return PRT_OK;
 }
 
-static void refit_commit_grid(PrtScene* s, const float origin[3], const float step[3], float coord_scale) {
+static void refit_commit_grid(PrtScene* s, const float origin[3], const float step[3], float coord_scale, bool bounded) {
     s->set_grid(origin, step, coord_scale);
+    s->bounded = bounded;
     ++s->generation;
 }
 
@@ -1606,7 +1613,7 @@
         float cs = std::max(g.root_hi[0], std::max(g.root_hi[1], g.root_hi[2]));
         if (s->bvh_info.built_on_device)
             for (int a = 0; a < 3; ++a) cs = std::max(cs, (float)(65535.0 * (double)step[a]));
-        refit_commit_grid(s, origin, step, std::nextafter(cs, std::numeric_limits<float>::infinity()));
+        refit_commit_grid(s, origin, step, std::nextafter(cs, std::numeric_limits<float>::infinity()), g.bounded);
     }
     PRT_HIP_AS(who, hipEventRecord(R.ev0.get(), st));
     launch_position_followers(s, d_verts, d_normals, g, st);
@@ -1667,7 +1674,7 @@
     }
     if ((rc = lights_then_readers(s, who, g.lights_moved, d_normals != nullptr, st))) return rc;
 
-    refit_commit_grid(s, db.grid_origin, db.grid_step, db.coord_scale);
+    refit_commit_grid(s, db.grid_origin, db.grid_step, db.coord_scale, g.bounded);
     const DTriShade* const shade_old = d.shade;
     const uint32_t* const order_old = s->d_order;
     DevBuf<> old[9] = {s->take(d.nodes),  s->take(s->d_order),        s->take(d.shade),      s->take(R.d_parent),
@@ -2484,8 +2491,9 @@
         P.items_per_chunk = pass.list_n;
     }
     const bool count = count_work != 0;
-    const bool plain = !generic_forced() && (f32 ? frame_plain(s, s->k32, count, pass.rays, P.jitter, P.scramble, P.sample_lights)
-                                                 : frame_plain(s, s->k64, count, pass.rays, P.jitter, P.scramble, P.sample_lights));
+    const bool bounded = frame_bounded(s, C);
+    const bool plain = !generic_forced() && (f32 ? frame_plain(s, s->k32, count, pass.rays, P.jitter, P.scramble, P.sample_lights, bounded)
+                                                 : frame_plain(s, s->k64, count, pass.rays, P.jitter, P.scramble, P.sample_lights, bounded));
     int bpc = (f32 ? s->k32.blocks_per_cu : s->k64.blocks_per_cu)[count ? 1 : plain ? 2 : 0];
     if (pass.rays) bpc = f32 ? rays_blocks_per_cu(s, s->k32) : rays_blocks_per_cu(s, s->k64);
     const uint64_t lanes = (uint64_t)s->n_cu * bpc * PRT_BLOCK;
@@ -2640,7 +2648,7 @@
     P.tile = 8; P.tiles_x = P.tiles_y = P.n_tiles = 1; P.rank = 0; P.nranks = 1; P.owned_tiles = 1;
     P.items_per_chunk = n_pixels;
     const bool count = trace != nullptr;
-    const bool plain = !generic_forced() && frame_plain(s, s->k64, count, false, P.jitter, P.scramble, P.sample_lights);
+    const bool plain = !generic_forced() && frame_plain(s, s->k64, count, false, P.jitter, P.scramble, P.sample_lights, frame_bounded(s, C));
     const int bpc = s->k64.blocks_per_cu[count ? 1 : plain ? 2 : 0];
     const size_t per_launch = n_pixels * (size_t)std::min<int>(sample_count, PRT_MAX_CHUNKS);
     Staging b;
diff --git a/pooraytracer_amd/csrc/prt_device.h b/pooraytracer_amd/csrc/prt_device.h
--- a/pooraytracer_amd/csrc/prt_device.h
+++ b/pooraytracer_amd/csrc/prt_device.h
@@ -15,6 +15,7 @@
 template <> struct real4_of<float> { typedef float4 type; };
 typedef real4_of<real>::type real4;
 #define PRT_NOCUR ((int32_t)0x80000000)
+#define PRT_PUSH_BIAS 3
 #ifndef PRT_BOX_PK
 #define PRT_BOX_PK 1
 #endif
@@ -78,6 +79,13 @@
 PRT_DEV float ieee_sqrt(float x) { return __builtin_amdgcn_sqrtf(x); }
 PRT_DEV double ieee_div(double a, double b) { return a / b; }
 PRT_DEV float ieee_div(float a, float b) { return a * __builtin_amdgcn_rcpf(b); }
+PRT_DEV double ieee_div_bounded(double a, double b) {
+    double r = __builtin_amdgcn_rcp(b);
+    r = fma(r, fma(-b, r, 1.0), r);
+    r = fma(r, fma(-b, r, 1.0), r);
+    const double q = a * r;
+    return fma(fma(-b, q, a), r, q);
+}
 PRT_DEV d3 operator/(d3 a, real s) {
     const real r = fast_rcp(s);
     return {a.x * r, a.y * r, a.z * r};
@@ -181,13 +189,17 @@
 }
 
 PRT_DEV real dot_yxz(real ax, real ay, real az, real bx, real by, real bz) { return fma(az, bz, fma(ax, bx, ay * by)); }
+template <bool BOUNDED = false>
 PRT_DEV bool tri_test_ord(const DTri* __restrict__ T, d3 o, d3 d, real tmin, real tmax, real& t_out, real& a_out,
                           real& b_out, const real4& q0, uint32_t* n_full) {
+    static_assert(!BOUNDED || !PRT_F32, "ieee_div_bounded is the fp64 sequence");
     const real4* q = reinterpret_cast<const real4*>(T);
     real4 q1 = q[1];
     real denom = dot_yxz(q0.x, q0.y, q0.z, d.x, d.y, d.z);
     if (fabs(denom) < RL(1e-8)) return false;
-    real t = ieee_div(q0.w - dot_yxz(q0.x, q0.y, q0.z, o.x, o.y, o.z), denom);
+    real t;
+    if constexpr (BOUNDED) t = ieee_div_bounded(q0.w - dot_yxz(q0.x, q0.y, q0.z, o.x, o.y, o.z), denom);
+    else t = ieee_div(q0.w - dot_yxz(q0.x, q0.y, q0.z, o.x, o.y, o.z), denom);
     if (!(tmin <= t && t <= tmax)) return false;
     if (n_full) ++*n_full;
     const real4 q2 = q[2];
@@ -280,7 +292,7 @@
         n = fmaxf(fmaxf(fmaxf(nx, ny), nz), tminf);
         f = fminf(fminf(fminf(fx, fy), fz), tbestf);
     }
-    template <bool COUNT>
+    template <bool COUNT, bool BIAS = false>
     PRT_DEV void inner_step(const DScene& S, uint32_t* stk, WorkCount& wc) {
         const uint4* np = reinterpret_cast<const uint4*>(reinterpret_cast<const char*>(S.nodes) + ((uint32_t)cur << 6));
         const uint4 bx = np[0], by = np[1], bz = np[2], rf = np[3];
@@ -313,15 +325,25 @@
 #undef PRT_CE
         const bool h1 = k1 != 0xffffffffu, h2 = k2 != 0xffffffffu, h3 = k3 != 0xffffffffu;
         sp += (int32_t)h1 + (int32_t)h2 + (int32_t)h3;
-        uint32_t* const top = stk + sp * 64;
-        if (h3) top[-3 * 64] = r3;
-        if (h2) top[-2 * 64] = r2;
-        if (h1) top[-1 * 64] = r1;
+        static_assert(PRT_PUSH_BIAS == 3, "the three pushes below");
+        if constexpr (BIAS) {
+            auto* low = (__attribute__((address_space(3))) uint32_t*)(stk + sp * 64);
+            asm volatile("" : "+v"(low));
+            if (h3) low[0 * 64] = r3;
+            if (h2) low[1 * 64] = r2;
+            if (h1) low[2 * 64] = r1;
+        } else {
+            uint32_t* const top = stk + sp * 64;
+            if (h3) top[-3 * 64] = r3;
+            if (h2) top[-2 * 64] = r2;
+            if (h1) top[-1 * 64] = r1;
+        }
         if (k0 != 0xffffffffu) {
             cur = (int32_t)r0;
         } else if (sp == 0) {
             cur = PRT_NOCUR;
         } else {
+            if constexpr (BIAS) stk += PRT_PUSH_BIAS * 64;
             sp--;
             cur = (int32_t)stk[sp * 64];
         }
@@ -353,7 +375,7 @@
         return stop;
     }
 
-    template <bool COUNT>
+    template <bool COUNT, bool BOUNDED = false>
     PRT_DEV bool test_leaf_pp(const DScene& S, int32_t ref, WorkCount& wc, real tmin_use, bool any_hit) {
         const uint32_t enc = ~(uint32_t)ref;
         const uint32_t first = enc >> 3, cnt = (enc & 7u) + 1u;
@@ -364,7 +386,7 @@
         auto test = [&](const real4& q0) {
             real t, al, be;
             if (COUNT) wc.tris++;
-            if (tri_test_ord(reinterpret_cast<const DTri*>(rec), o, d, tmin_use, hit.t, t, al, be, q0, COUNT ? &wc.tris_full : nullptr)) {
+            if (tri_test_ord<BOUNDED>(reinterpret_cast<const DTri*>(rec), o, d, tmin_use, hit.t, t, al, be, q0, COUNT ? &wc.tris_full : nullptr)) {
                 hit.t = t;
                 if (!any_hit) {
                     hit.alpha = al;
@@ -389,11 +411,12 @@
         return stop;
     }
 
-    template <bool COUNT, bool PP = false>
+    template <bool COUNT, bool PP = false, bool BIAS = false, bool BOUNDED = false>
     PRT_DEV void leaf_step(const DScene& S, uint32_t* stk, WorkCount& wc, real tmin_use, bool any_hit) {
+        static_assert(PP || !BOUNDED, "only test_leaf_pp has the bounded form");
         bool stop = false;
         if (cur < 0 && cur != PRT_NOCUR) {
-            if constexpr (PP) stop = test_leaf_pp<COUNT>(S, cur, wc, tmin_use, any_hit);
+            if constexpr (PP) stop = test_leaf_pp<COUNT, BOUNDED>(S, cur, wc, tmin_use, any_hit);
             else stop = test_leaf<COUNT>(S, cur, wc, tmin_use, any_hit);
             cur = PRT_NOCUR;
         }
@@ -402,6 +425,7 @@
         } else if (cur == PRT_NOCUR) {
             if (sp == 0) active = false;
             else {
+                if constexpr (BIAS) stk += PRT_PUSH_BIAS * 64;
                 sp--;
                 cur = (int32_t)stk[sp * 64];
             }
diff --git a/pooraytracer_amd/csrc/prt_host.h b/pooraytracer_amd/csrc/prt_host.h
--- a/pooraytracer_amd/csrc/prt_host.h
+++ b/pooraytracer_amd/csrc/prt_host.h
@@ -75,6 +75,9 @@
 void setup_triangles(const PrtSceneDesc& d, std::vector<HostTri>& out);
 void update_triangles(const double* vertices, const double* normals, std::vector<HostTri>& tris);
 void update_triangles_listed(const int32_t* prims, size_t n, const double* vertices, const double* normals, std::vector<HostTri>& tris);
+#define PRT_SCENE_BOUND 72057594037927936.0
+bool coords_bounded(const double* p, size_t n);
+bool scene_bounded(const std::vector<HostTri>& tris);
 void setup_materials(const PrtSceneDesc& d, std::vector<DMaterial>& out);
 bool build_bvh(const std::vector<HostTri>& tris, BuiltBVH& out, std::string* err);
 bool node_count_ok(size_t n_nodes, std::string* err);
diff --git a/pooraytracer_amd/csrc/prt_kernels.hip b/pooraytracer_amd/csrc/prt_kernels.hip
--- a/pooraytracer_amd/csrc/prt_kernels.hip
+++ b/pooraytracer_amd/csrc/prt_kernels.hip
@@ -291,6 +291,11 @@
 #define PARK_DIR_GLOBAL(feat) (((feat) & PRT_FEAT_TEX) != 0)
 #define PARK_AB_AT(feat) (PARK_DIR_GLOBAL(feat) ? PRT_RW + 1 : 4 * PRT_RW + 1)
 #define PARK_WORDS(feat) (((feat) & PRT_FEAT_TEX) ? 3 * PRT_RW + 1 : 4 * PRT_RW + 1)
+template <int WORDS>
+struct ParkedStacks {
+    uint32_t park[WORDS][PRT_BLOCK];
+    uint32_t stack[PRT_BLOCK / 64][PRT_STACK_DEPTH][64];
+};
 
 PRT_DEV void load_ray(const void* ray_list, uint32_t i, d3& o, d3& d) {
     const PrtRay* r = static_cast<const PrtRay*>(ray_list) + i;
@@ -332,7 +337,10 @@
     __shared__ real s_center[4];
     constexpr int NPARK = PRT_BLOCK;
     __shared__ uint32_t s_park[PARK_WORDS(FEAT)][NPARK];
-#define park (&s_park[0][threadIdx.x])
+    constexpr bool TRIM = PLAIN && !PRT_F32 && !PRT_DYN_STACK && PRT_ONE_PASS_VERTEX && !(FEAT & (PRT_FEAT_PHONG | PRT_FEAT_TEX));
+    __shared__ ParkedStacks<PARK_WORDS(FEAT)> s_lds;
+    static_assert(offsetof(ParkedStacks<PARK_WORDS(FEAT)>, stack) >= PRT_PUSH_BIAS * 64 * sizeof(uint32_t), "a biased stack column starts inside the object");
+#define park (TRIM ? &s_lds.park[0][threadIdx.x] : &s_park[0][threadIdx.x])
     const int lane = threadIdx.x & 63, wave = threadIdx.x >> 6;
     extern __shared__ __align__(16) unsigned char s_dyn_all[];
 #if PRT_DYN_STACK
@@ -340,7 +348,14 @@
     unsigned char* s_dyn = s_dyn_all + (size_t)(PRT_BLOCK / 64) * P.stack_depth * 64 * sizeof(uint32_t);
 #else
     __shared__ uint32_t s_stack[PRT_BLOCK / 64][PRT_STACK_DEPTH][64];
-    uint32_t* stk = &s_stack[wave][0][lane];
+    uint32_t* stk = TRIM ? reinterpret_cast<uint32_t*>(&s_lds) + (offsetof(ParkedStacks<PARK_WORDS(FEAT)>, stack) / sizeof(uint32_t) - PRT_PUSH_BIAS * 64) +
+                               (wave * PRT_STACK_DEPTH * 64 + lane)
+                         : &s_stack[wave][0][lane];
+    if constexpr (TRIM) {
+        auto* q = (__attribute__((address_space(3))) uint32_t*)stk;
+        asm volatile("" : "+v"(q));
+        stk = (uint32_t*)q;
+    }
     unsigned char* s_dyn = s_dyn_all;
 #endif
     if (lane == 0) {
@@ -418,6 +433,7 @@
     constexpr bool EVAL_FLAT = ONE_PASS && !(FEAT & PRT_FEAT_CT);
     constexpr bool TURN = ONE_PASS && PRT_SAMPLE_TURNOVER && !(PRT_F32 && !(FEAT & PRT_FEAT_CT));
     constexpr bool WAVE_DIET = ONE_PASS && !PRT_F32;
+    static_assert(TRIM == (PLAIN && WAVE_DIET && !PRT_DYN_STACK), "TRIM: the PLAIN forms of the WAVE_DIET kernels (said above, where the LDS is laid out)");
     d3 pending = mk3(0, 0, 0);
     d3 next_d = mk3(0, 0, 1);
     bool cont = false;
@@ -867,13 +883,13 @@
             if (!tr.active) tr.cur = PRT_NOCUR;
             do {
                 if (COUNT && lane_mask(tr.cur >= 0) != 0ULL) wc.inner_rounds++;
-                if (tr.cur >= 0) tr.template inner_step<COUNT>(S, stk, wc);
+                if (tr.cur >= 0) tr.template inner_step<COUNT, TRIM>(S, stk, wc);
                 const unsigned long long m_inner = lane_mask(tr.cur >= 0);
                 const unsigned long long m_parked = lane_mask((uint32_t)tr.cur > (uint32_t)PRT_NOCUR);
                 m_act = m_inner | m_parked;
                 if (__popcll(m_parked) >= P.leaf_batch || __popcll(m_inner) <= P.inner_min) {
                     if (COUNT && m_parked != 0ULL) wc.leaf_rounds++;
-                    if ((uint32_t)tr.cur > (uint32_t)PRT_NOCUR) tr.template leaf_step<COUNT, !COUNT>(S, stk, wc, sh ? RL(0.001) : RL(0.0001), sh);
+                    if ((uint32_t)tr.cur > (uint32_t)PRT_NOCUR) tr.template leaf_step<COUNT, !COUNT, TRIM, TRIM>(S, stk, wc, sh ? RL(0.001) : RL(0.0001), sh);
                     m_act = lane_mask(tr.cur != PRT_NOCUR);
                 }
                 const unsigned long long m_fin = m_chain & ~m_act;
@@ -1321,9 +1337,9 @@
 
 typedef void (*RenderKernel)(RenderArgs);
 constexpr bool plain_permutation(int perm) { return !PRT_F32_TU && perm != PRT_FEAT_TEX; }
-bool render_plain(int feat, bool count, bool rays, int n_lights, int ltri_lds, int jitter, int scramble, int sample_lights) {
+bool render_plain(int feat, bool count, bool rays, int n_lights, int ltri_lds, int jitter, int scramble, int sample_lights, bool bounded) {
     return plain_permutation(render_permutation(feat)) && !count && !rays && n_lights > 0 && ltri_lds > 0 && !jitter &&
-           scramble != PRT_ITEMS_FROM_LIST && sample_lights;
+           scramble != PRT_ITEMS_FROM_LIST && sample_lights && bounded;
 }
 template <int FEAT, bool PAD>
 static RenderKernel render_kernel_feat(bool count, bool llds, bool extra, bool rays, bool plain) {
diff --git a/pooraytracer_amd/csrc/prt_launch.h b/pooraytracer_amd/csrc/prt_launch.h
--- a/pooraytracer_amd/csrc/prt_launch.h
+++ b/pooraytracer_amd/csrc/prt_launch.h
@@ -9,7 +9,7 @@
 
 namespace prt {
 int render_blocks_per_cu(bool count, int feat, size_t table_bytes, int stack_depth, bool pad, bool extra, bool rays, bool plain);
-bool render_plain(int feat, bool count, bool rays, int n_lights, int ltri_lds, int jitter, int scramble, int sample_lights);
+bool render_plain(int feat, bool count, bool rays, int n_lights, int ltri_lds, int jitter, int scramble, int sample_lights, bool bounded);
 int render_permutation(int feat);
 int render_lds_budget(int feat, int stack_depth);
 size_t render_table_bytes(int light_lds, int mat_lds, int ltri_lds);
@@ -127,7 +127,7 @@
 
 namespace prt32 {
 int render_blocks_per_cu(bool count, int feat, size_t table_bytes, int stack_depth, bool pad, bool extra, bool rays, bool plain);
-bool render_plain(int feat, bool count, bool rays, int n_lights, int ltri_lds, int jitter, int scramble, int sample_lights);
+bool render_plain(int feat, bool count, bool rays, int n_lights, int ltri_lds, int jitter, int scramble, int sample_lights, bool bounded);
 int render_permutation(int feat);
 int render_lds_budget(int feat, int stack_depth);
 size_t render_table_bytes(int light_lds, int mat_lds, int ltri_lds);
diff --git a/pooraytracer_amd/csrc/scene_setup.cpp b/pooraytracer_amd/csrc/scene_setup.cpp
--- a/pooraytracer_amd/csrc/scene_setup.cpp
+++ b/pooraytracer_amd/csrc/scene_setup.cpp
@@ -112,6 +112,19 @@
         }
         setup_triangle_geometry(tris[t], p, vn);
     }
+}
+
+static bool all_below(const double* p, size_t n, double bound) {
+    for (size_t i = 0; i < n; ++i)
+        if (!(std::fabs(p[i]) < bound)) return false;
+    return true;
+}
+bool coords_bounded(const double* p, size_t n) { return all_below(p, n, PRT_SCENE_BOUND); }
+bool scene_bounded(const std::vector<HostTri>& tris) {
+    for (const HostTri& T : tris)
+        if (!all_below(&T.v[0][0], 9, PRT_SCENE_BOUND) || !all_below(T.normal, 3, 2.0 * PRT_SCENE_BOUND) || !all_below(&T.D, 1, 2.0 * PRT_SCENE_BOUND))
+            return false;
+    return true;
 }
 
 void setup_materials(const PrtSceneDesc& d, std::vector<DMaterial>& out) {
```

After: 14340 Mrays/s, median of 2. No clear change (-0.0%).
